# CMUAbstract/VINSat

Hardware: AMD Instinct MI355X
Metric: BA iterations/sec (500 poses, 50k landmarks) + final pose RMSE vs ref (higher is better)
Workload: dtype f64; 1 GPU; C3: 500-pose / 50000-observation window, 20-call schedule (10 landmark-only + 10 full); poses=500, observations=50000, windows_per_gpu=1, parallelism=replicas1, devices_visible=1, ranks_per_device=1

## Files before the change

### vinsat_amd/csrc/vba_api.hip

```cpp
#include "vba_context.h"

thread_local std::string g_err;

int fail(int code, const std::string& msg) {
    g_err = msg;
    return code;
}



void fill_params(StepParams& p, int iter, int initialize) {
    double alpha = 1.0 - (2.0 * ((double)iter / 5.0) - 1.0);
    alpha = std::min(std::max(alpha, 1.0), 2.0);
    const double it1 = (double)iter + 1.0;
    const double sigma = std::min(10000.0 * it1 * it1, 1000000.0);
    p.alpha = alpha;
    p.am2 = std::fabs(alpha - 2.0);
    p.expo = alpha / 2.0 - 1.0;
    p.alpha_is_2 = alpha == 2.0;
    p.sigma = sigma;
    p.sqrt_sigma = std::sqrt(sigma);
    p.initialize = initialize ? 1 : 0;
    p.iter = iter;
    p.pad = 0;
}

int check_window(vba_handle h, int window) {
    if (!h) return fail(VBA_EINVAL, "null handle");
    if (window < 0 || window >= h->W) return fail(VBA_EINVAL, "window index out of range");
    return VBA_OK;
}

int read_heads(vba_handle h) {
    HIPCHK(hipStreamSynchronize(h->stream));
    for (int w = 0; w < h->W; ++w)
        if (h->h_head[w].flags & 64u)
            return fail(VBA_ESTATE, "resident solve: a block of window " + std::to_string(w) + " timed out waiting for its producers (vba_set_fusion bits 5, 6)");
    return VBA_OK;
}

const volatile WinHead* head(vba_handle h, int w) { return h->h_head + w; }

hipError_t create_aux_stream(hipStream_t* s) {
    if (const char* m = std::getenv("VBA_AUX_CUMASK")) {
        const uint32_t word = (uint32_t)std::strtoul(m, nullptr, 16);
        uint32_t mask[8];
        for (auto& x : mask) x = word;
        return hipExtStreamCreateWithCUMask(s, 8, mask);
    }
    const char* e = std::getenv("VBA_AUX_PRIO");
    const int want = e ? std::atoi(e) : 0;
    if (want == 0) return hipStreamCreateWithFlags(s, hipStreamNonBlocking);
    int least = 0, greatest = 0;
    (void)hipDeviceGetStreamPriorityRange(&least, &greatest);
    return hipStreamCreateWithPriority(s, hipStreamNonBlocking, want > 0 ? greatest : least);
}

int settle(vba_handle h, bool boundary) {
    if (!h) return VBA_OK;
    if (!h->spec.valid) {
        if (boundary) h->prev_res_iter = -1;
        return VBA_OK;
    }
    HIPCHK(hipSetDevice(h->device));
    launch_reset_calls(h->V, h->stream);
    HIPCHK(hipGetLastError());
    HIPCHK(hipStreamSynchronize(h->stream));
    for (int w = 0; w < h->W; ++w) h->h_head[w].flags = 0;
    h->par = (h->chain_par0 + h->spec.c) & 1;
    h->carry_ok = 0;
    h->need_hist_reset = true;
    h->hist_dirty = false;
    h->spec.valid = false;
    h->spec_discards++;
    if (boundary && h->prev_res_iter >= 0) h->pred_iter[h->prev_res_iter & 63] = -2;
    h->prev_res_iter = -1;
    return VBA_OK;
}

int ready(vba_handle h) {
    for (int w = 0; w < h->W; ++w)
        if (!h->have_obs[w] || !h->have_win[w] || !h->have_state[w])
            return fail(VBA_ESTATE, "window " + std::to_string(w) + " is missing observations, pose constants or states");
    if (h->reg)
        for (int w = 0; w < h->W; ++w)
            if (!h->have_prior[w]) return fail(VBA_ESTATE, "window " + std::to_string(w) + " has no prior (vba_upload_prior)");
    return VBA_OK;
}



static int vba_set_accumulate_lanes(vba_handle h, int lanes);
static int vba_set_trial_tiles(vba_handle h, int tiles);
int vba_set_solver(vba_handle h, int chunk);

int vba_version(void) { return 230; }

const char* vba_last_error(void) { return g_err.c_str(); }

int vba_device_count(int* count) {
    if (!count) return fail(VBA_EINVAL, "null count");
    int c = 0;
    if (hipGetDeviceCount(&c) != hipSuccess) c = 0;
    *count = c;
    return VBA_OK;
}

constexpr int kLatWindowsCap = 192;
constexpr int kPartitionedWindowsMax = 1023;
static bool default_latency_mode(int windows, int64_t m_max) {
    const double x = m_max <= 50000 ? 0.7 : 0.46;
    return windows == 1 || (windows <= kLatWindowsCap && (double)windows <= 38.0 * std::pow(50000.0 / (double)m_max, x));
}
static int default_fusion(bool lat, int windows, int n_max, int64_t m_max) {
    const double rows = (double)windows * (double)m_max;
    if (windows == 1) return (lat && (m_max >= 150000 || n_max >= 1500)) ? 14 : 15;
    return !lat ? 15 : rows <= 175e3 ? 15 : rows <= 450e3 ? 14 : 12;
}

int vba_create(int device, int windows, int n_max, int64_t m_max, vba_handle* out) {
    return vba_create_mode(device, windows, n_max, m_max, -1, out);
}

int vba_create_mode(int device, int windows, int n_max, int64_t m_max, int mode, vba_handle* out) {
    if (!out) return fail(VBA_EINVAL, "null out");
    *out = nullptr;
    if (mode < -1 || mode > 1) return fail(VBA_EINVAL, "mode must be -1 (automatic), 0 (bandwidth-mode kernels) or 1 (latency-mode kernels)");
    const bool lat = mode == -1 ? default_latency_mode(windows, m_max) : mode == 1;
    if (windows < 1 || n_max < 2 || m_max < 1) return fail(VBA_EINVAL, "need windows >= 1, n_max >= 2, m_max >= 1");
    if (m_max > (int64_t)1 << 30) return fail(VBA_EINVAL, "m_max too large");
    int cnt = 0;
    if (hipGetDeviceCount(&cnt) != hipSuccess || cnt == 0) return fail(VBA_ENODEV, "no HIP device visible");
    if (device < 0 || device >= cnt) return fail(VBA_EINVAL, "device index out of range");
    HIPCHK(hipSetDevice(device));
    HIPCHK(configure_solver_device());
    vba_context* h = new (std::nothrow) vba_context();
    if (!h) return fail(VBA_ENOMEM, "host allocation failed");
    h->device = device;
    h->W = windows;
    h->n_max = n_max;
    h->m_max = m_max;
    const size_t W = windows, N = n_max, M = (size_t)m_max;
    const int nblk_obs = (int)((M + kObsBlock - 1) / kObsBlock);
    const int nblk_dyn = (int)((N + kObsBlock - 1) / kObsBlock);
    const int nblk_dyn16 = (int)((N - 1 + 14) / 15);
    const int trial_stride = nblk_obs + std::max(nblk_dyn, nblk_dyn16) + kLongCap;
    size_t bytes = 0;
    auto need = [&](size_t b) { bytes += ((b + 255) & ~size_t(255)) + 256; };
    need(W * 4); need(W * 4); need(W * sizeof(WinScalars));
    const size_t m_pad = (M + 31) & ~size_t(31);
    const size_t obs_stride = (6 * m_pad + m_pad / 2 + (N + 2) / 2 + 31) & ~size_t(31);
    need(W * obs_stride * 8);
    need(W * N * 10 * 8); need(W * N * 10 * 8);
    need(W * N * 4 * 8); need(W * N * 4 * 8); need(W * N * 4);
    const int nblk_pred = (int)((N * kDynLanes + 255) / 256);
    const int pred_stride = nblk_pred + kLongCap;
    need(W * 2 * pred_stride * 8); need(W * 2 * pred_stride * 8); need(W * 81 * 8);
    const size_t long_pool_cap = windows <= kLongPoolFewWindows ? kLongPoolFew : kLongPool;
    need(W * kLongCap * 4); need(W * 4); need(W * kLongCap * 4); need(W * 2 * long_pool_cap * 6 * 8);
    need(W * N * 36 * 8); need(W * N * 6 * 8);
    need(W * 2 * M * 8); need(2 * W * M * 8); need(W * 2 * M * 8); need(W * nblk_obs * 8); need(W * trial_stride * 8); need(W * nblk_obs * 8);
    need(W * kHistStride * 4);
    const int warm_shift = !lat ? 46 : (2 * m_max <= 300000 ? 44 : 43);
    int bucket_cap = 0;
    if (lat) {
        const double expect = 2.0 * (double)m_max * (warm_shift == 44 ? 0.0013 : 0.00065) * 6.0;
        bucket_cap = 256;
        while (bucket_cap < expect && bucket_cap < 4096) bucket_cap *= 2;
        need(W * 2 * (size_t)kSelBins * bucket_cap * 8);
    }
    const size_t per_pose = 2 * (21 + 6) + 2 * (6 + 36 + 6 + 1 + 3 + 9 + 9 + 9) + 243 + 9 + 81 + 9 + 9;
    need(W * N * per_pose * 8 + 16 * 256);
    need(W * N * 171 * 8);
    need(W * N * (171 + 171 + 81 + 9 + 9) * 8 + 6 * 256);
    need(W * N * (171 * 3 + 9) * 8 + 6 * 256);
    need(W * (N + 8) * 4);
    bytes += 1 << 16;
    if (hipMalloc(&h->arena.base, bytes) != hipSuccess) {
        delete h;
        return fail(VBA_ENOMEM, "hipMalloc of " + std::to_string(bytes) + " bytes failed");
    }
    h->arena.size = bytes;
    if (hipMemset(h->arena.base, 0, bytes) != hipSuccess || hipStreamSynchronize(nullptr) != hipSuccess) {
        hipFree(h->arena.base);
        delete h;
        return fail(VBA_EHIP, "hipMemset of the device arena failed");
    }
    Arena& A = h->arena;
    DevView& V = h->V;
    V.W = windows; V.n_max = n_max; V.m_max = m_max; V.nblk_obs = nblk_obs; V.nblk_dyn = nblk_dyn;
    V.n = h->d_n = A.take<int>(W);
    V.m = h->d_m = A.take<int>(W);
    V.sc = A.take<WinScalars>(W);
    h->d_obs = A.take<double>(W * obs_stride);
    h->m_pad = (int64_t)m_pad;
    V.obs_stride = (int64_t)obs_stride;
    V.ox = h->d_obs; V.oy = V.ox + m_pad; V.oz = V.oy + m_pad; V.ou = V.oz + m_pad; V.ov = V.ou + m_pad; V.oconf = V.ov + m_pad;
    V.opose = reinterpret_cast<const int*>(V.oconf + m_pad);
    V.pose_ptr = V.opose + m_pad;
    h->S[0] = A.take<double>(W * N * 10); h->S[1] = A.take<double>(W * N * 10);
    V.states = V.states_prev = h->S[0]; V.states_new = h->S[1];
    V.part_pred = A.take<double>(W * 2 * pred_stride); V.part_prior = A.take<double>(W * 2 * pred_stride); V.nblk_pred = nblk_pred;
    V.pred_stride = pred_stride;
    V.long_idx = h->d_long_idx = A.take<int>(W * kLongCap); V.n_long = h->d_n_long = A.take<int>(W);
    V.nblk_long = 0;
    V.long_off = h->d_long_off = A.take<int>(W * kLongCap);
    V.long_pool = A.take<double>(W * 2 * long_pool_cap * 6);
    V.long_pool_cap = (int)long_pool_cap;
    V.lastD = A.take<double>(W * 81);
    V.intr = h->d_intr = A.take<double>(W * N * 4);
    V.cumrot = h->d_cumrot = A.take<double>(W * N * 4);
    V.steps = h->d_steps = A.take<int>(W * N);
    V.prior_H = h->d_prior_H = A.take<double>(W * N * 36);
    V.prior_x = h->d_prior_x = A.take<double>(W * N * 6);
    V.reg = 0;
    V.absr = A.take<double>(W * 2 * M); V.wraw = h->wraw2 = A.take<double>(2 * W * M); V.ckeys = A.take<double>(W * 2 * M);
    V.acc_lanes = 8;
    V.part_init = A.take<double>(W * nblk_obs); V.part_trial = A.take<double>(W * trial_stride);
    V.trial_stride = trial_stride;
    V.part_next = A.take<double>(W * nblk_obs);
    V.hist = A.take<unsigned>(W * kHistStride);
    V.wbucket = bucket_cap ? A.take<double>(W * 2 * (size_t)kSelBins * bucket_cap) : nullptr;
    V.bucket_cap = bucket_cap;
    h->bucket_cap_alloc = bucket_cap;
    V.sel_inline = 0;
    V.Hraw = h->Hraw2 = A.take<double>(2 * W * N * 21); V.braw = h->braw2 = A.take<double>(2 * W * N * 6);
    V.xhat = h->dyn2[0] = A.take<double>(2 * W * N * 6); V.Phi = h->dyn2[1] = A.take<double>(2 * W * N * 36); V.rorb = h->dyn2[2] = A.take<double>(2 * W * N * 6);
    V.fatt = h->dyn2[3] = A.take<double>(2 * W * N); V.qgrad = h->dyn2[4] = A.take<double>(2 * W * N * 3);
    V.Hd = h->dyn2[5] = A.take<double>(2 * W * N * 9); V.Hu = h->dyn2[6] = A.take<double>(2 * W * N * 9); V.Hl = h->dyn2[7] = A.take<double>(2 * W * N * 9);
    V.bands = A.take<double>(W * N * 243); V.rhs = A.take<double>(W * N * 9);
    V.Xs = A.take<double>(W * N * 81); V.zs = A.take<double>(W * N * 9); V.dpose = A.take<double>(W * N * 9);
    V.p_max = n_max / 2 + 1;
    const size_t PM = V.p_max;
    V.csol = A.take<double>(W * N * 171);
    V.cL = A.take<double>(W * PM * 171); V.cR = A.take<double>(W * PM * 171);
    V.rXs = A.take<double>(W * PM * 81); V.rzs = A.take<double>(W * PM * 9); V.rx = A.take<double>(W * PM * 9);
    V.csol2 = A.take<double>(W * PM * 171); V.cL2 = A.take<double>(W * PM * 171); V.cR2 = A.take<double>(W * PM * 171);
    V.rx2 = A.take<double>(W * PM * 9);
    V.res_stride = n_max + 8;
    V.res_flags = A.take<unsigned>(W * (N + 8));
    V.resident = 0;
    V.m_total = 0; V.abs_all = nullptr; V.abs_all_count = 0;
    V.hop = 0; V.pivot = 0; V.call = -1; V.emit = 0; V.carry = 0; V.dyn_in_acc = 0;
    V.par = 0; V.fold = 0; V.redo = 0; V.fused_trial = 0; V.pending_only = 0; V.warm_force_miss = 0;
    V.lat = lat ? 1 : 0;
    V.trial_tiles = 1;
    V.warm_shift = warm_shift;
    V.chunk = 0; V.chunk2 = 0;
    {
        const void* must[] = {V.n, V.m, V.sc, V.ox, V.oy, V.oz, V.ou, V.ov, V.oconf, V.opose, V.pose_ptr, V.states,
                              V.states_new, V.states_prev, V.intr, V.cumrot, V.steps, V.prior_H, V.prior_x, V.absr, V.wraw, V.ckeys, V.part_init, V.part_next,
                              V.part_pred, V.part_prior, V.lastD, V.long_idx, V.n_long, V.long_off, V.long_pool,
                              V.part_trial, V.hist, V.Hraw, V.braw, V.xhat, V.Phi, V.rorb, V.fatt, V.qgrad, V.Hd, V.Hu, V.Hl,
                              V.bands, V.rhs, V.Xs, V.zs, V.dpose, V.csol, V.cL, V.cR, V.rXs, V.rzs, V.rx, V.csol2, V.cL2, V.cR2, V.rx2, V.res_flags};
        bool ok = A.used <= A.size;
        for (const void* q : must) ok = ok && q != nullptr;
        if (!ok) {
            hipFree(A.base);
            delete h;
            return fail(VBA_ENOMEM, "internal: device arena mis-carved");
        }
    }
    for (int k = 0; k < 64; ++k) h->pred_iter[k] = h->pred_init[k] = -1;
    h->V.host_states = nullptr;
    h->fusion = default_fusion(lat, windows, n_max, m_max);
    if ((windows == 1 && (hipEventCreateWithFlags(&h->ev_first, hipEventDisableTiming) != hipSuccess ||
                          hipHostMalloc((void**)&h->h_states_map, (size_t)2 * n_max * 10 * sizeof(double), hipHostMallocMapped | hipHostMallocCoherent) != hipSuccess ||
                          hipHostGetDevicePointer((void**)&h->V.host_states, h->h_states_map, 0) != hipSuccess)) ||
        hipStreamCreateWithFlags(&h->own_stream, hipStreamNonBlocking) != hipSuccess ||
        (!lat && create_aux_stream(&h->aux_stream) != hipSuccess) ||
        hipEventCreate(&h->ev0) != hipSuccess || hipEventCreate(&h->ev1) != hipSuccess ||
        hipEventCreateWithFlags(&h->ev_fork, hipEventDisableTiming) != hipSuccess ||
        hipEventCreateWithFlags(&h->ev_join, hipEventDisableTiming) != hipSuccess ||
        hipEventCreateWithFlags(&h->ev_stage, hipEventDisableTiming) != hipSuccess ||
        hipEventCreateWithFlags(&h->ev_up[0], hipEventDisableTiming) != hipSuccess ||
        hipEventCreateWithFlags(&h->ev_up[1], hipEventDisableTiming) != hipSuccess ||
        hipHostMalloc((void**)&h->h_up[0], std::max(obs_stride, 9 * N + 160) * sizeof(double), hipHostMallocDefault) != hipSuccess ||
        hipHostMalloc((void**)&h->h_up[1], std::max(obs_stride, 9 * N + 160) * sizeof(double), hipHostMallocDefault) != hipSuccess ||
        hipHostMalloc((void**)&h->h_stage, ((size_t)n_max * 10 + 1) * sizeof(double), hipHostMallocDefault) != hipSuccess ||
        hipHostMalloc((void**)&h->h_back, (size_t)n_max * 10 * sizeof(double) + sizeof(WinScalars), hipHostMallocDefault) != hipSuccess ||
        hipHostMalloc((void**)&h->h_head, W * sizeof(WinHead), hipHostMallocMapped | hipHostMallocCoherent) != hipSuccess ||
        hipHostGetDevicePointer((void**)&h->V.host_head, h->h_head, 0) != hipSuccess) {
        vba_destroy(h);
        return fail(VBA_EHIP, "stream/event/pinned allocation failed");
    }
    h->stream = h->own_stream;
    h->n.assign(W, 0); h->m.assign(W, 0); h->n_long.assign(W, 0);
    h->have_obs.assign(W, 0); h->have_win.assign(W, 0); h->have_state.assign(W, 0); h->have_prior.assign(W, 0);
    h->perm.resize(W);
    vba_set_accumulate_lanes(h, 0);
    vba_set_trial_tiles(h, 0);
    vba_set_solver(h, -1);
    h->warm_enabled = 1;
    h->fold_enabled = lat;
    if (const char* e = std::getenv("VBA_X_FOLD")) h->fold_enabled = std::atoi(e) != 0;
#ifdef VBA_VARIANTS
    if (const char* e = std::getenv("VBA_CR_LEVELS")) h->cr_levels = std::atoi(e) == 3 ? 3 : 2;
#endif
    *out = h;
    return VBA_OK;
}

int vba_has_variants(void) {
#ifdef VBA_VARIANTS
    return 1;
#else
    return 0;
#endif
}

int vba_get_mode(vba_handle h, int* mode, int* chunk) {
    if (!h) return fail(VBA_EINVAL, "null handle");
    if (mode) *mode = h->V.lat;
    if (chunk) *chunk = h->V.chunk;
    return VBA_OK;
}

int vba_destroy(vba_handle h) {
    if (!h) return VBA_OK;
    (void)settle(h);
    watch_stop(h);
    hipSetDevice(h->device);
    (void)vba_sh_comm_destroy(h);
    if (h->own_stream) { hipStreamSynchronize(h->own_stream); hipStreamDestroy(h->own_stream); }
    if (h->aux_stream) { hipStreamSynchronize(h->aux_stream); hipStreamDestroy(h->aux_stream); }
    for (hipEvent_t e : h->cprof.ev) if (e) hipEventDestroy(e);
    for (auto& ge : h->graphs) if (ge.exec) (void)hipGraphExecDestroy(ge.exec);
    if (h->ev_first) hipEventDestroy(h->ev_first);
    if (h->h_states_map) hipHostFree(h->h_states_map);
    if (h->ev_fork) hipEventDestroy(h->ev_fork);
    if (h->ev_join) hipEventDestroy(h->ev_join);
    if (h->ev0) hipEventDestroy(h->ev0);
    if (h->ev1) hipEventDestroy(h->ev1);
    if (h->ev_stage) hipEventDestroy(h->ev_stage);
    for (int k = 0; k < 2; ++k) {
        if (h->ev_up[k]) hipEventDestroy(h->ev_up[k]);
        if (h->h_up[k]) hipHostFree(h->h_up[k]);
    }
    if (h->h_stage) hipHostFree(h->h_stage);
    if (h->h_back) hipHostFree(h->h_back);
    if (h->h_head) hipHostFree(h->h_head);
    if (h->d_dbg) hipFree(h->d_dbg);
    for (QueryScratch* q : {&h->q_cov, &h->q_rel, &h->q_pow}) {
        if (q->d) hipFree(q->d);
        if (q->ev) hipEventDestroy(q->ev);
    }
    if (h->cov_ev0) hipEventDestroy(h->cov_ev0);
    if (h->arena.base) hipFree(h->arena.base);
    delete h;
    return VBA_OK;
}

int vba_set_solver2(vba_handle h, int chunk, int chunk2) {
    if (!h) return fail(VBA_EINVAL, "null handle");
    if (int rc_settle = settle(h)) return rc_settle;
    if (chunk < 2 || chunk > 60 || (chunk2 != 0 && chunk2 != -1 && (chunk2 < 2 || chunk2 > 60)))
        return fail(VBA_EINVAL, "chunk sizes must be in [2, 60] (chunk2 = 0: single level, -1: cyclic reduction)");
    if (chunk2 == -1 && (h->n_max + chunk - 1) / chunk - 1 > 128)
        return fail(VBA_EINVAL, "chunk2 = -1 needs at most 128 separators: chunk >= ceil(n_max / 129)");
    h->V.chunk = chunk;
    h->V.chunk2 = chunk2;
    h->no_pack = 0;
    return VBA_OK;
}

int vba_set_solver(vba_handle h, int chunk) {
    if (!h) return fail(VBA_EINVAL, "null handle");
    if (int rc_settle = settle(h)) return rc_settle;
    h->V.chunk2 = 0;
    if (chunk == -1) {
        h->no_pack = 0;
        if (h->W > kPartitionedWindowsMax || h->n_max < 8) { h->V.chunk = 0; return VBA_OK; }
        const int c64 = (h->n_max + 64) / 65, c128 = (h->n_max + 128) / 129;
        int c1 = std::max(std::min(c64, std::max(8, c128)), 2);
        if (!h->V.lat) c1 = std::max(c1, std::min(12, std::max(2, h->n_max / 3)));
        if (h->V.lat) c1 = std::max(c1, std::min(8, std::max(2, h->n_max / 3)));
        if (h->V.lat && h->W > 1) {
            int c = c1;
            while (c < 12 && (int64_t)h->W * ((h->n_max + c - 1) / c) > 1024) ++c;
            if ((int64_t)h->W * ((h->n_max + c - 1) / c) <= 1024) c1 = c;
        }
        if (c1 <= 60) {
            h->V.chunk = c1;
            h->V.chunk2 = -1;
        } else {
            const int c3 = std::min(std::max((int)std::ceil(std::cbrt((double)h->n_max)), 2), 60);
            h->V.chunk = c3;
            h->V.chunk2 = c3;
        }
        return VBA_OK;
    }
    if (chunk == -2) {
        h->V.chunk = 0;
        h->no_pack = 1;
        return VBA_OK;
    }
#ifndef VBA_VARIANTS
    if (chunk == -3) return fail(VBA_EINVAL, "three windows per wavefront (k_solve_packed) is a comparison variant that this build does not carry (make VARIANTS=1)");
#endif
    if (chunk == -3) {
        h->V.chunk = 0;
        h->no_pack = 0;
        h->pack_min = 3;
        return VBA_OK;
    }
    if (chunk < 0 || chunk == 1 || chunk > 60) return fail(VBA_EINVAL, "chunk must be -3, -2, -1, 0 or in [2, 60]");
    h->V.chunk = chunk;
    h->no_pack = 0;
    return VBA_OK;
}

int vba_set_integrator(vba_handle h, int hop100) {
    if (!h) return fail(VBA_EINVAL, "null handle");
    if (int rc_settle = settle(h)) return rc_settle;
    h->V.hop = hop100 ? 1 : 0;
    h->V.nblk_long = h->V.hop ? 0 : *std::max_element(h->n_long.begin(), h->n_long.end());
    return VBA_OK;
}

static int vba_set_accumulate_lanes(vba_handle h, int lanes) {
    if (!h) return fail(VBA_EINVAL, "null handle");
    if (int rc_settle = settle(h)) return rc_settle;
    if (lanes == 0) {
        const double avg = (double)h->m_max / (double)h->n_max;
        int G = 4;
        while (G < 64 && avg / G > 16.0) G *= 2;
        while (G < 64 && (int64_t)h->W * h->n_max * G * 2 <= 49152) G *= 2;
        lanes = G;
    }
    if (lanes != 4 && lanes != 8 && lanes != 16 && lanes != 32 && lanes != 64) return fail(VBA_EINVAL, "lanes must be 0, 4, 8, 16, 32 or 64");
    h->V.acc_lanes = lanes;
    return VBA_OK;
}

static int vba_set_trial_tiles(vba_handle h, int tiles) {
    if (!h) return fail(VBA_EINVAL, "null handle");
    if (int rc_settle = settle(h)) return rc_settle;
    if (tiles == 0) {
        const int64_t blocks = (int64_t)h->W * h->V.nblk_obs;
        tiles = blocks >= 600 ? 4 : (blocks >= 150 ? 2 : 1);
    }
    if (tiles != 1 && tiles != 2 && tiles != 4 && tiles != 8) return fail(VBA_EINVAL, "tiles must be 0 (automatic), 1, 2, 4 or 8");
    h->V.trial_tiles = tiles;
    return VBA_OK;
}

static int vba_set_key_carry(vba_handle h, int on) {
    if (!h) return fail(VBA_EINVAL, "null handle");
    if (int rc_settle = settle(h)) return rc_settle;
    h->carry_enabled = on != 0;
    h->carry_ok = false;
    return VBA_OK;
}

static int vba_set_fusion(vba_handle h, int mask) {
    if (!h) return fail(VBA_EINVAL, "null handle");
    if (int rc_settle = settle(h)) return rc_settle;
    if (mask < 0 || mask > 127) return fail(VBA_EINVAL, "mask must be in [0, 127]");
#ifndef VBA_VARIANTS
    if (mask & (16 | 32 | 64)) return fail(VBA_EINVAL, "mask bits 4 .. 6 select comparison variants that this build does not carry (make VARIANTS=1)");
#endif
    h->fusion = mask;
    h->fusion_auto = false;
    return VBA_OK;
}

static int vba_set_chunk_waves(vba_handle h, int waves) {
    if (!h) return fail(VBA_EINVAL, "null handle");
    if (int rc_settle = settle(h)) return rc_settle;
    if (waves != 1 && waves != 2) return fail(VBA_EINVAL, "waves must be 1 or 2");
    h->chunk_waves = waves;
    return VBA_OK;
}

static int vba_set_warm_select(vba_handle h, int on) {
    if (!h) return fail(VBA_EINVAL, "null handle");
    if (int rc_settle = settle(h)) return rc_settle;
    h->warm_enabled = on == 2 ? 2 : (on != 0);
    h->inline_select = on != 3;
    return VBA_OK;
}

static int vba_set_warm_shift(vba_handle h, int shift) {
    if (!h) return fail(VBA_EINVAL, "null handle");
    if (int rc_settle = settle(h)) return rc_settle;
    if (shift < 42 || shift > 51) return fail(VBA_EINVAL, "shift must be in [42, 51]");
    h->V.warm_shift = shift;
    h->carry_ok = 0;
    return VBA_OK;
}

static int vba_set_bucket_cap(vba_handle h, int cap) {
    if (!h) return fail(VBA_EINVAL, "null handle");
    if (int rc_settle = settle(h)) return rc_settle;
    if (!h->bucket_cap_alloc) return fail(VBA_ESTATE, "this handle has no bin buckets (16 windows or more)");
    if (cap != 0 && (cap < 8 || cap > h->bucket_cap_alloc)) return fail(VBA_EINVAL, "cap must be 0 (default) or in [8, allocated capacity]");
    h->V.bucket_cap = cap ? cap : h->bucket_cap_alloc;
    h->carry_ok = 0;
    return VBA_OK;
}

int vba_set_host_watch(vba_handle h, int slot, const void* live, const void* copy, int64_t bytes) {
    if (!h || slot < 0 || slot >= 8) return fail(VBA_EINVAL, "bad argument (8 watch slots)");
    if (live && (!copy || bytes < 1)) return fail(VBA_EINVAL, "a watched buffer needs its reference copy and a size");
    watch_quiesce(h);
    h->watch[slot].live = live;
    h->watch[slot].copy = live ? copy : nullptr;
    h->watch[slot].bytes = live ? (size_t)bytes : 0;
    return VBA_OK;
}

static int vba_set_pipeline(vba_handle h, int on) {
    if (!h) return fail(VBA_EINVAL, "null handle");
    if (int rc = settle(h)) return rc;
    h->pipeline = on != 0;
    return VBA_OK;
}

int vba_pipeline_stats(vba_handle h, int* hits, int* discards) {
    if (!h) return fail(VBA_EINVAL, "null handle");
    if (hits) *hits = h->spec_hits;
    if (discards) *discards = h->spec_discards;
    return VBA_OK;
}

int vba_warm_select_misses(vba_handle h, int* count) {
    if (!h || !count) return fail(VBA_EINVAL, "null argument");
    *count = h->warm_misses;
    return VBA_OK;
}

static int vba_set_jacobian_f32(vba_handle h, int on) {
    if (!h) return fail(VBA_EINVAL, "null handle");
    if (int rc_settle = settle(h)) return rc_settle;
    if (on != 0 && on != 1) return fail(VBA_EINVAL, "jacobian_f32 must be 0 (fp64, default) or 1 (fp32)");
    h->V.jac_f32 = on;
    return VBA_OK;
}

static int vba_set_pivoting(vba_handle h, int always) {
    if (!h) return fail(VBA_EINVAL, "null handle");
    if (int rc_settle = settle(h)) return rc_settle;
    h->pivot_mode = always ? 1 : 0;
    return VBA_OK;
}

int vba_solver_fallbacks(vba_handle h, int* count) {
    if (!h || !count) return fail(VBA_EINVAL, "null argument");
    *count = h->fallbacks;
    return VBA_OK;
}

int vba_set_stream(vba_handle h, void* hip_stream, int external) {
    if (!h) return fail(VBA_EINVAL, "null handle");
    if (int rc_settle = settle(h)) return rc_settle;
    hipStreamSynchronize(h->stream);
    h->stream = external ? (hipStream_t)hip_stream : h->own_stream;
    return VBA_OK;
}

int vba_upload_observations(vba_handle h, int window, int n, int64_t m, const double* xyz, const double* uv,
                            const double* conf, const int64_t* ii) {
    if (int rc = check_window(h, window)) return rc;
    if (int rc_settle = settle(h, true)) return rc_settle;
    if (!xyz || !uv || !conf || !ii) return fail(VBA_EINVAL, "null observation array");
    h->carry_ok = false;
    if (n < 2 || n > h->n_max) return fail(VBA_EINVAL, "n out of range (need 2 <= n <= n_max)");
    if (m < 1 || m > h->m_max) return fail(VBA_EINVAL, "m out of range (need 1 <= m <= m_max)");
    if (h->have_win[window] && h->n[window] != n) { h->have_win[window] = 0; h->have_state[window] = 0; h->have_prior[window] = 0; }
    HIPCHK(hipSetDevice(h->device));
    std::vector<int> ptr(n + 1, 0);
    for (int64_t k = 0; k < m; ++k) {
        if (ii[k] < 0 || ii[k] >= n) return fail(VBA_EINVAL, "ii[" + std::to_string(k) + "] outside [0, n)");
        ptr[ii[k] + 1]++;
    }
    for (int i = 0; i < n; ++i) ptr[i + 1] += ptr[i];
    std::vector<int64_t>& perm = h->perm[window];
    perm.assign(m, 0);
    if (!h->perm_stale.empty()) h->perm_stale[window] = 1;
    {
        std::vector<int> cur(ptr.begin(), ptr.end() - 1);
        for (int64_t k = 0; k < m; ++k) perm[cur[ii[k]]++] = k;
    }
    const int ub = h->up_next;
    h->up_next ^= 1;
    HIPCHK(hipEventSynchronize(h->ev_up[ub]));
    double* blk = h->h_up[ub];
    const size_t mp = (size_t)h->m_pad;
    double *x = blk, *y = x + mp, *z = y + mp, *u = z + mp, *v = u + mp, *c = v + mp;
    int* pose = reinterpret_cast<int*>(c + mp);
    int* cptr = pose + mp;
    for (int64_t s = 0; s < m; ++s) {
        const int64_t k = perm[s];
        x[s] = xyz[3 * k]; y[s] = xyz[3 * k + 1]; z[s] = xyz[3 * k + 2];
        u[s] = uv[2 * k]; v[s] = uv[2 * k + 1];
        c[s] = conf[k];
        pose[s] = (int)ii[k];
    }
    std::memcpy(cptr, ptr.data(), (size_t)(n + 1) * sizeof(int));
    const int mi = (int)m;
    const size_t used = (size_t)(reinterpret_cast<char*>(cptr + n + 1) - reinterpret_cast<char*>(blk));
    HIPCHK(hipMemcpyAsync(h->d_obs + (size_t)window * h->V.obs_stride, blk, used, hipMemcpyHostToDevice, h->stream));
    HIPCHK(hipEventRecord(h->ev_up[ub], h->stream));
    launch_set_counts(h->V, window, n, mi, h->stream);
    HIPCHK(hipGetLastError());
    h->n[window] = n;
    h->m[window] = mi;
    h->have_obs[window] = 1;
    h->V.n_min = *std::min_element(h->n.begin(), h->n.end());
    return VBA_OK;
}

int vba_upload_window(vba_handle h, int window, int n, const double* intrinsics, const double* cumrot_last,
                      const int64_t* time_idx) {
    if (int rc = check_window(h, window)) return rc;
    if (int rc_settle = settle(h, true)) return rc_settle;
    if (!intrinsics || !cumrot_last || !time_idx) return fail(VBA_EINVAL, "null pose-constant array");
    h->carry_ok = false;
    if (n < 2 || n > h->n_max) return fail(VBA_EINVAL, "n out of range (need 2 <= n <= n_max)");
    if (h->have_obs[window] && h->n[window] != n) { h->have_obs[window] = 0; h->have_state[window] = 0; h->have_prior[window] = 0; }
    HIPCHK(hipSetDevice(h->device));
    std::vector<int> steps(n);
    for (int i = 0; i + 1 < n; ++i) {
        const int64_t d = time_idx[i + 1] - time_idx[i];
        if (d < 1) return fail(VBA_EINVAL, "time_idx must be strictly increasing");
        if (d > VBA_MAX_GAP) return fail(VBA_EINVAL, "time_idx: a gap longer than VBA_MAX_GAP (2^20 s)");
        steps[i] = (int)d;
    }
    steps[n - 1] = 1;
    int long_list[2 * kLongCap + 1];
    int nl = 0, pool_used = 0;
    for (int i = 0; i + 1 < n && nl < kLongCap; ++i)
        if (steps[i] > kLongGap) {
            const int need_states = long_pool_states(long_plan(steps[i]));
            if (pool_used + need_states > h->V.long_pool_cap) continue;
            long_list[kLongCap + 1 + nl] = pool_used;
            pool_used += need_states;
            long_list[nl++] = i;
            steps[i] = -steps[i];
        }
    long_list[kLongCap] = nl;
    const size_t pb = (size_t)window * h->n_max;
    const int ub = h->up_next;
    h->up_next ^= 1;
    HIPCHK(hipEventSynchronize(h->ev_up[ub]));
    double* blk = h->h_up[ub];
    std::memcpy(blk, intrinsics, (size_t)n * 32);
    std::memcpy(blk + (size_t)n * 4, cumrot_last, (size_t)n * 32);
    std::memcpy(blk + (size_t)n * 8, steps.data(), (size_t)n * 4);
    double* lblk = blk + (size_t)n * 8 + (size_t)(n + 1) / 2;
    std::memcpy(lblk, long_list, sizeof(long_list));
    HIPCHK(hipMemcpyAsync(h->d_intr + pb * 4, blk, (size_t)n * 32, hipMemcpyHostToDevice, h->stream));
    HIPCHK(hipMemcpyAsync(h->d_cumrot + pb * 4, blk + (size_t)n * 4, (size_t)n * 32, hipMemcpyHostToDevice, h->stream));
    HIPCHK(hipMemcpyAsync(h->d_steps + pb, blk + (size_t)n * 8, (size_t)n * 4, hipMemcpyHostToDevice, h->stream));
    if (nl) {
        HIPCHK(hipMemcpyAsync(h->d_long_idx + (size_t)window * kLongCap, lblk, (size_t)nl * 4, hipMemcpyHostToDevice, h->stream));
        HIPCHK(hipMemcpyAsync(h->d_long_off + (size_t)window * kLongCap, reinterpret_cast<const int*>(lblk) + kLongCap + 1, (size_t)nl * 4,
                              hipMemcpyHostToDevice, h->stream));
    }
    HIPCHK(hipMemcpyAsync(h->d_n_long + window, reinterpret_cast<const int*>(lblk) + kLongCap, 4, hipMemcpyHostToDevice, h->stream));
    if (nl || h->n_long[window])
        HIPCHK(hipMemsetAsync(h->V.long_pool + (size_t)window * 2 * h->V.long_pool_cap * 6, 0xFF,
                              (size_t)2 * h->V.long_pool_cap * 6 * sizeof(double), h->stream));
    HIPCHK(hipEventRecord(h->ev_up[ub], h->stream));
    h->n_long[window] = nl;
    h->V.nblk_long = h->V.hop ? 0 : *std::max_element(h->n_long.begin(), h->n_long.end());
    launch_set_counts(h->V, window, n, -1, h->stream);
    HIPCHK(hipGetLastError());
    h->n[window] = n;
    h->have_win[window] = 1;
    return VBA_OK;
}

int vba_upload_prior(vba_handle h, int window, int n, const double* states_prior, const double* hessian_state) {
    if (int rc = check_window(h, window)) return rc;
    if (int rc_settle = settle(h, true)) return rc_settle;
    if (!states_prior || !hessian_state) return fail(VBA_EINVAL, "null prior array");
    if (!h->have_obs[window] && !h->have_win[window]) return fail(VBA_ESTATE, "upload the window before its prior");
    if (n != h->n[window]) return fail(VBA_EINVAL, "the prior needs one row per pose of the window");
    HIPCHK(hipSetDevice(h->device));
    std::vector<double> xp((size_t)n * 6);
    for (int i = 0; i < n; ++i) {
        const double* s = states_prior + (size_t)i * 10;
        double* o = xp.data() + (size_t)i * 6;
        o[0] = s[0]; o[1] = s[1]; o[2] = s[2]; o[3] = s[7]; o[4] = s[8]; o[5] = s[9];
    }
    HIPCHK(hipStreamSynchronize(h->stream));
    const size_t pb = (size_t)window * h->n_max;
    HIPCHK(hipMemcpy(h->d_prior_x + pb * 6, xp.data(), xp.size() * 8, hipMemcpyHostToDevice));
    HIPCHK(hipMemcpy(h->d_prior_H + pb * 36, hessian_state, (size_t)n * 36 * 8, hipMemcpyHostToDevice));
    h->have_prior[window] = 1;
    return VBA_OK;
}

int vba_set_prior(vba_handle h, int on) {
    if (!h) return fail(VBA_EINVAL, "null handle");
    h->reg = on != 0;
    return VBA_OK;
}

int vba_set_states(vba_handle h, int window, const double* states, double lamda) {
    if (!h) return fail(VBA_EINVAL, "null handle");
    if (int rc_settle = settle(h, true)) return rc_settle;
    if (!states) return fail(VBA_EINVAL, "null states");
    h->carry_ok = 0;
    double* S = h->S[h->par];
    if (window == -1) {
        const int n = h->n[0];
        for (int w = 0; w < h->W; ++w) {
            if (!h->have_obs[w] && !h->have_win[w]) return fail(VBA_ESTATE, "upload the windows before their states");
            if (h->n[w] != n) return fail(VBA_EINVAL, "window = -1 needs equal pose counts");
        }
        HIPCHK(hipSetDevice(h->device));
        HIPCHK(hipEventSynchronize(h->ev_stage));
        std::memcpy(h->h_stage, states, (size_t)n * 80);
        HIPCHK(hipMemcpyAsync(S, h->h_stage, (size_t)n * 80, hipMemcpyHostToDevice, h->stream));
        HIPCHK(hipEventRecord(h->ev_stage, h->stream));
        DevView V = h->V;
        V.states = S;
        V.par = h->par;
        launch_broadcast_states(V, n, lamda, h->stream);
        HIPCHK(hipGetLastError());
        for (int w = 0; w < h->W; ++w) h->have_state[w] = 1;
        return VBA_OK;
    }
    if (int rc = check_window(h, window)) return rc;
    if (!h->have_obs[window] && !h->have_win[window]) return fail(VBA_ESTATE, "upload the window before its states");
    HIPCHK(hipSetDevice(h->device));
    const int n = h->n[window];
    HIPCHK(hipEventSynchronize(h->ev_stage));
    std::memcpy(h->h_stage, states, (size_t)n * 80);
    h->h_stage[(size_t)h->n_max * 10] = lamda;
    HIPCHK(hipMemcpyAsync(S + (size_t)window * h->n_max * 10, h->h_stage, (size_t)n * 80, hipMemcpyHostToDevice, h->stream));
    HIPCHK(hipMemcpyAsync(&h->V.sc[window].lam[h->par], h->h_stage + (size_t)h->n_max * 10, 8, hipMemcpyHostToDevice, h->stream));
    HIPCHK(hipEventRecord(h->ev_stage, h->stream));
    h->have_state[window] = 1;
    return VBA_OK;
}

void unpack_scalars(const WinScalars* sc, int par, double* lamda, double* last_hessian, int* n_trials, unsigned* flags) {
    if (lamda) *lamda = sc->lam[par];
    if (last_hessian) std::memcpy(last_hessian, sc->last_hessian, 81 * 8);
    if (n_trials) *n_trials = sc->n_trials;
    if (flags) *flags = sc->fl[par ^ 1] & 7u;
}

int vba_get_states(vba_handle h, int window, double* states, double* lamda, double* last_hessian, int* n_trials,
                   unsigned* flags) {
    if (int rc = check_window(h, window)) return rc;
    if (int rc_settle = settle(h)) return rc_settle;
    if (!h->have_state[window]) return fail(VBA_ESTATE, "no states uploaded");
    HIPCHK(hipSetDevice(h->device));
    const int n = h->n[window];
    WinScalars* sc = reinterpret_cast<WinScalars*>(h->h_back + (size_t)h->n_max * 10);
    if (states) HIPCHK(hipMemcpyAsync(h->h_back, h->S[h->par] + (size_t)window * h->n_max * 10, (size_t)n * 80, hipMemcpyDeviceToHost, h->stream));
    HIPCHK(hipMemcpyAsync(sc, h->V.sc + window, sizeof(WinScalars), hipMemcpyDeviceToHost, h->stream));
    HIPCHK(hipStreamSynchronize(h->stream));
    if (states) std::memcpy(states, h->h_back, (size_t)n * 80);
    unpack_scalars(sc, h->par, lamda, last_hessian, n_trials, flags);
    return VBA_OK;
}

int vba_set_states_all(vba_handle h, const double* states, const double* lamda) {
    if (!h) return fail(VBA_EINVAL, "null handle");
    if (int rc_settle = settle(h, true)) return rc_settle;
    if (!states || !lamda) return fail(VBA_EINVAL, "null states / lamda");
    for (int w = 0; w < h->W; ++w)
        if (!h->have_obs[w] && !h->have_win[w]) return fail(VBA_ESTATE, "upload the windows before their states");
    HIPCHK(hipSetDevice(h->device));
    h->carry_ok = 0;
    const size_t per = (size_t)h->n_max * 10;
    HIPCHK(hipStreamSynchronize(h->stream));
    HIPCHK(hipMemcpy(h->S[h->par], states, (size_t)h->W * per * sizeof(double), hipMemcpyHostToDevice));
    std::vector<WinScalars> sc((size_t)h->W);
    HIPCHK(hipMemcpy(sc.data(), h->V.sc, sc.size() * sizeof(WinScalars), hipMemcpyDeviceToHost));
    for (int w = 0; w < h->W; ++w) sc[w].lam[h->par] = lamda[w];
    HIPCHK(hipMemcpy(h->V.sc, sc.data(), sc.size() * sizeof(WinScalars), hipMemcpyHostToDevice));
    for (int w = 0; w < h->W; ++w) h->have_state[w] = 1;
    return VBA_OK;
}

int vba_get_states_all(vba_handle h, double* states, double* lamda, double* last_hessian, int* n_trials, unsigned* flags) {
    if (!h) return fail(VBA_EINVAL, "null handle");
    if (int rc_settle = settle(h)) return rc_settle;
    for (int w = 0; w < h->W; ++w)
        if (!h->have_state[w]) return fail(VBA_ESTATE, "no states uploaded");
    HIPCHK(hipSetDevice(h->device));
    HIPCHK(hipStreamSynchronize(h->stream));
    const size_t per = (size_t)h->n_max * 10;
    if (states) HIPCHK(hipMemcpy(states, h->S[h->par], (size_t)h->W * per * sizeof(double), hipMemcpyDeviceToHost));
    std::vector<WinScalars> sc((size_t)h->W);
    HIPCHK(hipMemcpy(sc.data(), h->V.sc, sc.size() * sizeof(WinScalars), hipMemcpyDeviceToHost));
    for (int w = 0; w < h->W; ++w)
        unpack_scalars(&sc[w], h->par, lamda ? lamda + w : nullptr, last_hessian ? last_hessian + (size_t)w * 81 : nullptr,
                       n_trials ? n_trials + w : nullptr, flags ? flags + w : nullptr);
    return VBA_OK;
}


int vba_set_option(vba_handle h, int option, int value) {
    switch (option) {
        case VBA_OPT_ACCUMULATE_LANES: return vba_set_accumulate_lanes(h, value);
        case VBA_OPT_TRIAL_TILES: return vba_set_trial_tiles(h, value);
        case VBA_OPT_KEY_CARRY: return vba_set_key_carry(h, value);
        case VBA_OPT_WARM_SELECT: return vba_set_warm_select(h, value);
        case VBA_OPT_WARM_SHIFT: return vba_set_warm_shift(h, value);
        case VBA_OPT_BUCKET_CAP: return vba_set_bucket_cap(h, value);
        case VBA_OPT_FUSION: return vba_set_fusion(h, value);
        case VBA_OPT_CHUNK_WAVES: return vba_set_chunk_waves(h, value);
        case VBA_OPT_PIVOTING: return vba_set_pivoting(h, value);
        case VBA_OPT_PIPELINE: return vba_set_pipeline(h, value);
        case VBA_OPT_SCHEDULE_GRAPH: return vba_set_schedule_graph(h, value);
        case VBA_OPT_CHAIN_PROFILE: return vba_set_chain_profile(h, value);
        case VBA_OPT_JACOBIAN_F32: return vba_set_jacobian_f32(h, value);
        default: return fail(VBA_EINVAL, "unknown option (VBA_OPT_*)");
    }
}

int vba_last_step_ms(vba_handle h, float* ms) {
    if (!h || !ms) return fail(VBA_EINVAL, "null argument");
    if (!h->stepped) return fail(VBA_ESTATE, "no step has run");
    *ms = h->last_ms;
    return VBA_OK;
}

int vba_debug_fetch(vba_handle h, int window, int what, double* out, int64_t capacity, int64_t* count) {
    if (int rc = check_window(h, window)) return rc;
    if (int rc_settle = settle(h)) return rc_settle;
    if (!out || !count) return fail(VBA_EINVAL, "null output");
    if (!h->stepped) return fail(VBA_ESTATE, "no step has run");
    if (h->last_pipelined)
        return fail(VBA_ESTATE, "the last call was a pipelined vba_iterate_resident: the call speculated behind it has reused its scratch "
                                "(maximum weight, step, trial states); switch the pipeline off (vba_set_pipeline(h, 0)) to inspect intermediates");
    HIPCHK(hipSetDevice(h->device));
    HIPCHK(hipStreamSynchronize(h->stream));
    const int n = h->n[window];
    const int64_t m = h->m[window];
    const size_t pb = (size_t)window * h->n_max;
    DevView V;
    {
        CallSpec c;
        c.iter = h->last_iter; c.initialize = h->last_init; c.call = -1; c.par = h->par ^ 1;
        view_for_call(h, V, c);
    }
    auto copy = [&](const double* src, int64_t cnt) -> int {
        if (cnt > capacity) return fail(VBA_EINVAL, "debug buffer too small");
        HIPCHK(hipMemcpy(out, src, cnt * 8, hipMemcpyDeviceToHost));
        *count = cnt;
        return VBA_OK;
    };
    WinScalars sc;
    HIPCHK(hipMemcpy(&sc, V.sc + window, sizeof(sc), hipMemcpyDeviceToHost));
    double wmax;
    std::memcpy(&wmax, &sc.wmax_bits[V.par], 8);
    switch (what) {
#ifdef VBA_RESIDENT_STAMPS
        case 100:
            return copy(V.cR2 + (size_t)window * V.res_stride * 4, (int64_t)V.res_stride * 4);
        case 102: {
            if (capacity < 64) return fail(VBA_EINVAL, "debug buffer too small");
            fetch_ostamps(reinterpret_cast<unsigned long long*>(out));
            *count = 64;
            return VBA_OK;
        }
        case 101: {
            if (capacity < 128) return fail(VBA_EINVAL, "debug buffer too small");
            fetch_kstamps(reinterpret_cast<unsigned long long*>(out));
            *count = 128;
            return VBA_OK;
        }
#endif
        case VBA_DBG_EST:
        case VBA_DBG_WEIGHT:
        case VBA_DBG_JG: {
            const int64_t per = what == VBA_DBG_EST ? 2 : (what == VBA_DBG_JG ? 12 : 1);
            if (m * per > capacity) return fail(VBA_EINVAL, "debug buffer too small");
            const size_t need = (size_t)m * 15 * 8;
            if (h->dbg_cap < need) {
                if (h->d_dbg) hipFree(h->d_dbg);
                h->d_dbg = nullptr;
                h->dbg_cap = 0;
                HIPCHK(hipMalloc(&h->d_dbg, need));
                h->dbg_cap = need;
            }
            double* est = h->d_dbg;
            double* J = est + 2 * m;
            double* wt = J + 12 * m;
            launch_debug_project(V, window, (int)m, est, J, wt, h->stream);
            HIPCHK(hipGetLastError());
            HIPCHK(hipStreamSynchronize(h->stream));
            std::vector<double> tmp((size_t)m * per);
            const double* src = what == VBA_DBG_EST ? est : (what == VBA_DBG_JG ? J : wt);
            HIPCHK(hipMemcpy(tmp.data(), src, (size_t)m * per * 8, hipMemcpyDeviceToHost));
            const std::vector<int64_t>& perm = h->perm[window];
            for (int64_t s = 0; s < m; ++s) std::memcpy(out + perm[s] * per, tmp.data() + s * per, per * 8);
            *count = m * per;
            return VBA_OK;
        }
        case VBA_DBG_H: {
            if ((int64_t)n * 36 > capacity) return fail(VBA_EINVAL, "debug buffer too small");
            std::vector<double> tmp((size_t)n * 21);
            HIPCHK(hipMemcpy(tmp.data(), V.Hraw + pb * 21, (size_t)n * 21 * 8, hipMemcpyDeviceToHost));
            for (int i = 0; i < n; ++i)
                for (int a = 0; a < 6; ++a)
                    for (int b = 0; b < 6; ++b) out[(size_t)i * 36 + a * 6 + b] = tmp[(size_t)i * 21 + sym6(a, b)] / wmax;
            *count = (int64_t)n * 36;
            return VBA_OK;
        }
        case VBA_DBG_B: {
            if (int rc = copy(V.braw + pb * 6, (int64_t)n * 6)) return rc;
            for (int64_t k = 0; k < (int64_t)n * 6; ++k) out[k] /= wmax;
            return VBA_OK;
        }
        case VBA_DBG_PHI: return copy(V.Phi + pb * 36, (int64_t)n * 36);
        case VBA_DBG_RPRED: {
            if ((int64_t)(n - 1) * 7 > capacity) return fail(VBA_EINVAL, "debug buffer too small");
            std::vector<double> ro((size_t)n * 6), fa(n);
            HIPCHK(hipMemcpy(ro.data(), V.rorb + pb * 6, (size_t)n * 48, hipMemcpyDeviceToHost));
            HIPCHK(hipMemcpy(fa.data(), V.fatt + pb, (size_t)n * 8, hipMemcpyDeviceToHost));
            for (int i = 0; i < n - 1; ++i) {
                for (int r = 0; r < 6; ++r) out[(size_t)i * 7 + r] = ro[(size_t)i * 6 + r];
                out[(size_t)i * 7 + 6] = fa[i];
            }
            *count = (int64_t)(n - 1) * 7;
            return VBA_OK;
        }
        case VBA_DBG_QGRAD: return copy(V.qgrad + pb * 3, (int64_t)n * 3);
        case VBA_DBG_HQ: {
            if ((int64_t)n * 27 > capacity) return fail(VBA_EINVAL, "debug buffer too small");
            std::vector<double> d((size_t)n * 9), u((size_t)n * 9), l((size_t)n * 9);
            HIPCHK(hipMemcpy(d.data(), V.Hd + pb * 9, (size_t)n * 72, hipMemcpyDeviceToHost));
            HIPCHK(hipMemcpy(u.data(), V.Hu + pb * 9, (size_t)n * 72, hipMemcpyDeviceToHost));
            HIPCHK(hipMemcpy(l.data(), V.Hl + pb * 9, (size_t)n * 72, hipMemcpyDeviceToHost));
            for (int i = 0; i < n; ++i)
                for (int k = 0; k < 9; ++k) {
                    out[(size_t)i * 27 + k] = l[(size_t)i * 9 + k];
                    out[(size_t)i * 27 + 9 + k] = d[(size_t)i * 9 + k];
                    out[(size_t)i * 27 + 18 + k] = u[(size_t)i * 9 + k];
                }
            *count = (int64_t)n * 27;
            return VBA_OK;
        }
        case VBA_DBG_BANDS: {
            if (!std::getenv("VBA_DBG_RAW_BANDS")) launch_assemble(V, 0, h->stream);
            HIPCHK(hipGetLastError());
            HIPCHK(hipStreamSynchronize(h->stream));
            if (int rc = copy(V.bands + pb * 243, (int64_t)n * 243)) return rc;
            if (h->last_init) {
                for (int i = 0; i < n; ++i) {
                    std::memset(out + (size_t)i * 243, 0, 81 * 8);
                    std::memset(out + (size_t)i * 243 + 162, 0, 81 * 8);
                }
            }
            return VBA_OK;
        }
        case VBA_DBG_RHS: {
            if (!std::getenv("VBA_DBG_RAW_BANDS")) launch_assemble(V, 0, h->stream);
            HIPCHK(hipGetLastError());
            HIPCHK(hipStreamSynchronize(h->stream));
            return copy(V.rhs + pb * 9, (int64_t)n * 9);
        }
        case VBA_DBG_DPOSE: return copy(V.dpose + pb * 9, (int64_t)n * 9);
        case VBA_DBG_SCALARS: {
            if (capacity < 8) return fail(VBA_EINVAL, "debug buffer too small");
            StepParams p;
            fill_params(p, h->last_iter, h->last_init);
            out[0] = sc.c_obs; out[1] = wmax; out[2] = sc.init_residual; out[3] = sc.trial_residual;
            out[4] = sc.lam32; out[5] = p.sigma; out[6] = p.alpha; out[7] = (double)sc.n_trials;
            *count = 8;
            return VBA_OK;
        }
        default: return fail(VBA_EINVAL, "unknown debug selector");
    }
}
```

### vinsat_amd/csrc/vba_context.h

```cpp
#pragma once
#include <algorithm>
#include <atomic>
#include <chrono>
#include <cmath>
#include <condition_variable>
#include <mutex>
#include <thread>
#include <cstdio>
#include <cstdlib>
#include <cstring>
#include <new>
#include <string>
#include <vector>

#include <dlfcn.h>
#include <unistd.h>
#include <rccl/rccl.h>

#include "../../include/vinsat_ba.h"
#include "vba_device.h"
#include "vba_launch.h"
#include "vba_query_layout.h"

using namespace vba;

#pragma GCC visibility push(hidden)
extern thread_local std::string g_err;
int fail(int code, const std::string& msg);
#define HIPCHK(expr)                                                                                   \
    do {                                                                                               \
        hipError_t e_ = (expr);                                                                        \
        if (e_ != hipSuccess)                                                                          \
            return fail(VBA_EHIP, std::string(#expr) + ": " + hipGetErrorString(e_));                  \
    } while (0)

struct Arena {
    char* base = nullptr;
    size_t size = 0, used = 0;
    template <class T>
    T* take(size_t count) {
        used = (used + 255) & ~size_t(255);
        T* p = reinterpret_cast<T*>(base + used);
        used += count * sizeof(T);
        return p;
    }
};

struct QueryScratch {
    void* d = nullptr;
    size_t cap = 0;
    hipEvent_t ev = nullptr;
    float ms = 0.f;
    bool ran = false;
};

struct vba_context {
    int device = 0;
    int W = 0, n_max = 0;
    int64_t m_max = 0;
    hipStream_t own_stream = nullptr, stream = nullptr, aux_stream = nullptr;
    hipEvent_t ev0 = nullptr, ev1 = nullptr, ev_fork = nullptr, ev_join = nullptr;
    Arena arena;
    DevView V{};
    int *d_n = nullptr, *d_m = nullptr, *d_steps = nullptr;
    int *d_long_idx = nullptr, *d_n_long = nullptr, *d_long_off = nullptr;
    std::vector<int> n_long;
    double *wraw2 = nullptr, *Hraw2 = nullptr, *braw2 = nullptr;
    double* dyn2[8] = {};
    double* d_obs = nullptr;
    int64_t m_pad = 0;
    double *d_intr = nullptr, *d_cumrot = nullptr;
    double* h_up[2] = {nullptr, nullptr};
    hipEvent_t ev_up[2] = {nullptr, nullptr};
    int up_next = 0;
    WinHead* h_head = nullptr;
    double* h_stage = nullptr;
    double* h_back = nullptr;
    bool back_valid = false;
    double* S[2] = {nullptr, nullptr};
    int par = 0;
    bool need_hist_reset = false;
    hipEvent_t ev_stage = nullptr;
    std::vector<int> n, m;
    std::vector<char> have_obs, have_win, have_state, have_prior;
    bool reg = false;
    double *d_prior_H = nullptr, *d_prior_x = nullptr;
    std::vector<std::vector<int64_t>> perm;
    float last_ms = 0.f;
    bool stepped = false;
    int carry_ok = 0;
    bool carry_enabled = true;
    bool hist_dirty = false;
    bool fold_enabled = true;
    int warm_enabled = 1;
    int last_iter = 0, last_init = 0;
    int sh_pivot = 0;
    bool sh_rode = false, sh_bands_ready = false;
    struct ShComm {
        void* dl = nullptr;
        ncclComm_t comm = nullptr;
        int nranks = 0, rank = 0;
        ncclResult_t (*all_gather)(const void*, void*, size_t, ncclDataType_t, ncclComm_t, hipStream_t) = nullptr;
        ncclResult_t (*comm_destroy)(ncclComm_t) = nullptr;
        const char* (*error_string)(ncclResult_t) = nullptr;
        double* buf = nullptr;
        int64_t m_total = 0, m_pad = 0;
        int n = 0;
        int m_local = -1;
        int protocol = 1;
        ncclResult_t (*group_start)() = nullptr;
        ncclResult_t (*group_end)() = nullptr;
        double* buf2 = nullptr;
        int lenA = 0, lenB = 0, n2 = 0, nbo2 = 0, nbd2 = 0, cap2 = 0;
        double *sendA[2] = {nullptr, nullptr}, *recvA = nullptr, *sendB = nullptr, *recvB = nullptr;
        bool carried = false;
        int carried_par = 0;
        long fallbacks_miss = 0, fallbacks_lm = 0;
        double *abs_local = nullptr, *abs_all = nullptr, *partial_local = nullptr, *partial_all = nullptr, *trial_local = nullptr, *trial_all = nullptr;
    } shc;
    int pack_min = 1 << 30;
    int no_pack = 0;
    int pivot_mode = 0;
    int fallbacks = 0;
    int inline_select = 1;
    int chunk_waves = 2;
    int cr_levels = 2;
    int fusion = 15;
    bool fusion_auto = true;
    struct GraphEntry { std::vector<unsigned long long> key; std::vector<unsigned char> views; hipGraphExec_t exec = nullptr; };
    std::vector<GraphEntry> graphs;
    bool graph_broken = false;
    bool graph_enabled = true;
    long graph_replays = 0, graph_captures = 0;
    int bucket_cap_alloc = 0;
    int warm_misses = 0;
    double* d_dbg = nullptr;
    size_t dbg_cap = 0;
    QueryScratch q_cov;
    QueryScratch q_rel;
    QueryScratch q_pow;
    hipEvent_t cov_ev0 = nullptr;
    bool sharded = false;
    std::vector<char> perm_stale;
    struct Spec { bool valid = false; int iter = 0, init = 0; bool reg = false; int c = 0; } spec;
    int chain_par0 = 0;
    int pred_iter[64], pred_init[64];
    int prev_res_iter = -1;
    int pipeline = 1;
    bool last_pipelined = false;
    int spec_hits = 0, spec_discards = 0;
    struct Watch { const void* live = nullptr; const void* copy = nullptr; size_t bytes = 0; } watch[8];
    struct WatchWorker {
        std::thread th;
        std::mutex m;
        std::condition_variable cv;
        unsigned long long seq = 0;
        bool quit = false;
        std::atomic<unsigned long long> done_seq{0};
        bool changed = false;
        bool started = false;
        pid_t owner = 0;
    } ww;
    struct ChainProf {
        bool on = false;
        std::vector<hipEvent_t> ev;
        double ms[3] = {0.0, 0.0, 0.0};
        int64_t launches[3] = {0, 0, 0};
    } cprof;
    double* h_states_map = nullptr;
    hipEvent_t ev_first = nullptr;
};

void fill_params(StepParams& p, int iter, int initialize);
int check_window(vba_handle h, int window);
int read_heads(vba_handle h);
const volatile WinHead* head(vba_handle h, int w);
hipError_t create_aux_stream(hipStream_t* s);
int settle(vba_handle h, bool boundary = false);
int ready(vba_handle h);
void unpack_scalars(const WinScalars* sc, int par, double* lamda, double* last_hessian, int* n_trials, unsigned* flags);

struct CallSpec {
    bool host_out = false;
    int iter = 0, initialize = 0;
    int call = -1;
    int par = 0;
    int carry = 0;
    int emit = 0;
    bool fold = false;
    bool prof = false;
};

struct CallCtx {
    DevView V;
    hipEvent_t after_first = nullptr;
    bool fuse_assemble = false;
    bool assembled = false;
    bool bands_ready = false;
};

void view_for_call(vba_handle h, DevView& V, const CallSpec& c);
int enqueue_front(vba_handle h, CallCtx& C, const CallSpec& c, bool exact_repeat, hipEvent_t* ev);
void enqueue_trial(vba_handle h, CallCtx& C, const CallSpec& c, bool first, hipEvent_t ev_solve = nullptr, int solve_redo = -1);
int step_impl(vba_handle h, int iter, int initialize, float* prof, bool emit = true, int readback = -1);
void watch_stop(vba_handle h);
void watch_quiesce(vba_handle h);
int vba_set_schedule_graph(vba_handle h, int on);
int vba_set_chain_profile(vba_handle h, int on);

struct CovQuery {
    DevView V;
    double* diag = nullptr;
    double* sup = nullptr;
    unsigned* flags = nullptr;
};
int cov_begin(vba_handle h, int iter, const char* who);
int cov_build_invert(vba_handle h, int iter, int damped, CovQuery& q);
int query_reserve(vba_handle h, QueryScratch& q, size_t bytes, const char* what);
int query_finish(vba_handle h, QueryScratch& q);
int query_last_ms(vba_handle h, QueryScratch vba_context::*q, float* ms, const char* none_ran);

int rel_device_perm(vba_handle h, const int** d_perm);
int query_copy_out(double* out, const double* dev, size_t W, size_t stride, const std::vector<int>& used, size_t per);
#pragma GCC visibility pop
```

### vinsat_amd/csrc/vba_launch.h

```cpp
#pragma once
#include <hip/hip_runtime.h>

#include "vba_device.h"

namespace vba {

void launch_obs_residual(const DevView& V, double* abs_out, hipStream_t s);
void launch_select(const DevView& V, bool with_digit0, hipStream_t s);
void launch_select_warm(const DevView& V, hipStream_t s);
void launch_select_finish(const DevView& V, hipStream_t s);
void launch_obs_accumulate(const DevView& V, hipStream_t s);
void launch_trial(const DevView& V, hipStream_t s);
void launch_clear_hist(const DevView& V, int which, hipStream_t s);
void launch_reset_calls(const DevView& V, hipStream_t s);
void launch_set_counts(const DevView& V, int w, int n, int m, hipStream_t s);
void launch_broadcast_states(const DevView& V, int n, double lamda, hipStream_t s);
void launch_debug_project(const DevView& V, int w, int m, double* est, double* J, double* wt, hipStream_t s);

void launch_sh_clear_miss(const DevView& V, hipStream_t s);
void launch_sh_front(const DevView& V, const double* gathered, int ranks, int slot_len, double* bucket_out, int do_fold, int do_resolve, hipStream_t s);

void launch_dynamics(const DevView& V, hipStream_t s);
void launch_assemble(const DevView& V, int fuse_init_solve, hipStream_t s);

void launch_long_factor(const DevView& V, hipStream_t s);
void launch_long_trial(const DevView& V, hipStream_t s);

void launch_solve(const DevView& V, int initialize, hipStream_t s);
#ifdef VBA_RESIDENT_STAMPS
void fetch_kstamps(unsigned long long* out);
void fetch_ostamps(unsigned long long* out);
#endif
hipError_t configure_solver_device();
bool solve_forms_blocks(const DevView& V);
void launch_decide(const DevView& V, const double* trial_all, int ranks, hipStream_t s);

void launch_shard_pack(const DevView& V, double* partial_out, hipStream_t s);
void launch_shard_reduce(const DevView& V, const double* partial_all, int ranks, hipStream_t s, int with_sum = 1);
void launch_shard_trial_sum(const DevView& V, double* trial_local, hipStream_t s);

}
```

### vinsat_amd/csrc/vba_obs.hip

```cpp
#include "vba_decide.h"
#include <cstdlib>
#include "vba_device.h"
#include "vba_dyn_body.h"
#include "vba_launch.h"
#include "vba_step.h"

namespace vba {

__device__ __forceinline__ void begin_call_scalars(WinScalars& sc, int par, bool keep_wmax = false) {
    sc.done = 0;
    sc.n_trials = 0;
    sc.fl[par] = 0u;
    if (!keep_wmax) sc.wmax_bits[par] = 0ull;
    sc.sum_abs_rpred = 0.0;
}

template <bool HIST0>
__global__ __launch_bounds__(kObsBlock) void k_obs_residual(DevView V, double* abs_out ) {
    __shared__ double red[kObsBlock / 64];
    __shared__ unsigned lh[HIST0 ? 1024 : 1];
    const int w = blockIdx.y;
    VBA_SKIP_CALL(V, w);
    const int m = V.m[w];
    const size_t ob = (size_t)w * V.obs_stride;
    const size_t mb = (size_t)w * V.m_max;
    const int k = blockIdx.x * kObsBlock + threadIdx.x;
    if (HIST0) {
        for (int b = threadIdx.x; b < 1024; b += kObsBlock) lh[b] = 0u;
        __syncthreads();
    }
    double s = 0.0;
    if (k < m) {
        const int pose = V.opose[2 * ob + k];
        const size_t pb = (size_t)w * V.n_max + pose;
        PoseCam pc;
        pose_camera(V.states + pb * 10, V.intr + pb * 4, pc);
        double u, v, cam[3], d;
        project(pc, V.ox[ob + k], V.oy[ob + k], V.oz[ob + k], u, v, cam, d);
        const double ru = fabs(V.ou[ob + k] - u), rv = fabs(V.ov[ob + k] - v);
        double* ab = abs_out ? abs_out : V.absr + 2 * mb;
        reinterpret_cast<double2*>(ab)[k] = make_double2(ru, rv);
        s = ru + rv;
        if (HIST0) {
            atomicAdd(&lh[(unsigned)(f64_bits(ru) >> 53) & 1023u], 1u);
            atomicAdd(&lh[(unsigned)(f64_bits(rv) >> 53) & 1023u], 1u);
        }
    }
    const double t = block_sum<kObsBlock>(s, red);
    if (threadIdx.x == 0) V.part_init[(size_t)w * V.nblk_obs + blockIdx.x] = t;
    if (blockIdx.x == 0 && threadIdx.x == 0) {
        begin_call_scalars(V.sc[w], V.par);
        V.sc[w].sel_cnt = 0u;
    }
    if (HIST0) {
        unsigned* hist = hist0_of(V, w, V.par);
        for (int b = threadIdx.x; b < 1024; b += kObsBlock) {
            const unsigned c = lh[b];
            if (c) atomicAdd(&hist[b], c);
        }
        if (blockIdx.x == 0 && threadIdx.x == 0) {
            V.sc[w].sel_prefix[0] = 0ull;
            V.sc[w].sel_rank[0] = (2 * (long long)m - 1) / 2;
        }
    }
}

template <int P, bool COMPACT, int ITEMS>
__global__ __launch_bounds__(256) void k_select_pass(DevView V) {
    __shared__ unsigned lh[kSelBins];
    __shared__ unsigned lds_u[260];
    __shared__ double red[kObsBlock / 64];
    const int w = blockIdx.y;
    VBA_SKIP_CALL(V, w);
    const double* keys = V.abs_all ? V.abs_all : V.absr + 2 * (size_t)w * V.m_max;
    const int64_t count = V.abs_all ? V.abs_all_count : 2 * (int64_t)V.m[w];
    if (P == 1 && V.carry && blockIdx.x == 0 && threadIdx.x == 0) {
        begin_call_scalars(V.sc[w], V.par);
        V.sc[w].sel_cnt = 0u;
    }
    if (P == 1 && !V.carry && V.m_total == 0 && blockIdx.x == 0) {
        const double* pi = V.part_init + (size_t)w * V.nblk_obs;
        double s_init = 0.0;
        for (int b = threadIdx.x; b < V.nblk_obs; b += 256) s_init += pi[b];
        const double tot = block_sum<256>(s_init, red);
        if (threadIdx.x == 0) V.sc[w].sum_in[V.par] = tot;
    }
    if ((int64_t)blockIdx.x * 256 * ITEMS >= count) return;
    auto digit_hist = [&](int d) { return d == 0 ? hist0_of(V, w, V.par) : histd_of(V, w, d); };
    constexpr int nbins = 1 << sel_width(P);
    for (int b = threadIdx.x; b < nbins; b += 256) lh[b] = 0u;
    constexpr bool PRELOAD = ITEMS <= 8;
    constexpr int PAIRS = ITEMS / 2;
    const double2* keys2 = reinterpret_cast<const double2*>(keys);
    const int64_t npair = count / 2;
    double2 pk[PRELOAD ? PAIRS : 1];
    if (PRELOAD) {
#pragma unroll
        for (int it = 0; it < PAIRS; ++it) {
            const int64_t idx = ((int64_t)blockIdx.x * PAIRS + it) * 256 + threadIdx.x;
            pk[it] = idx < npair ? keys2[idx] : make_double2(0.0, 0.0);
        }
    }
    unsigned long long prefix = 0ull;
    long long rank = ((V.m_total ? 2 * V.m_total : count) - 1) / 2;
    if (P > 0) {
        constexpr int Q = P > 0 ? P - 1 : 0;
        select_resolve(digit_hist(Q), 1 << sel_width(Q), sel_width(Q), V.sc[w].sel_prefix[Q], V.sc[w].sel_rank[Q],
                       prefix, rank, lds_u);
    } else {
        __syncthreads();
    }
    if (blockIdx.x == 0 && threadIdx.x == 0) {
        V.sc[w].sel_prefix[P] = prefix;
        V.sc[w].sel_rank[P] = rank;
        if (COMPACT) V.sc[w].sel_mode = 0;
    }
    auto take = [&](unsigned long long key, bool have) {
        bool match = have;
        if (P > 0) match = have && (key >> sel_shift(P > 0 ? P - 1 : 0)) == prefix;
        if (match) atomicAdd(&lh[(unsigned)(key >> sel_shift(P)) & (nbins - 1)], 1u);
        if (COMPACT) {
            const unsigned long long mask = __ballot(match);
            if (mask) {
                const int lane = threadIdx.x & 63;
                const int leader = __ffsll((long long)mask) - 1;
                unsigned base = 0;
                if (lane == leader) base = atomicAdd(&V.sc[w].sel_cnt, (unsigned)__popcll(mask));
                base = (unsigned)__builtin_amdgcn_readlane((int)base, leader);
                if (match) {
                    const unsigned off = (unsigned)__popcll(mask & ((1ull << lane) - 1ull));
                    if ((int64_t)base + off < 2 * V.m_max) V.ckeys[2 * (size_t)w * V.m_max + base + off] = bits_f64(key);
                }
            }
        }
    };
#pragma unroll 8
    for (int it = 0; it < PAIRS; ++it) {
        const int64_t idx = ((int64_t)blockIdx.x * PAIRS + it) * 256 + threadIdx.x;
        const bool have = idx < npair;
        const double2 kk = PRELOAD ? pk[it] : (have ? keys2[idx] : make_double2(0.0, 0.0));
        take(f64_bits(kk.x), have);
        take(f64_bits(kk.y), have);
    }
    __syncthreads();
    unsigned* hist_out = digit_hist(P);
    for (int b = threadIdx.x; b < nbins; b += 256) {
        const unsigned c = lh[b];
        if (c) atomicAdd(&hist_out[b], c);
    }
}

enum { kWarmSkip = 0, kWarmHit = 1, kWarmMiss = 2 };

__device__ __forceinline__ bool fold_decide(const DevView& V, int w, double (*red)[4], DecideOut& d) {
    d = decide_eval(V, w, V.par ^ 1, V.prev, 0, 0.0, nullptr, 0, red);
    return d.accept && !(d.flags & (2u | 8u | 32u));
}
__device__ __forceinline__ DecideIn fold_load(const DevView& V, int w) { return decide_load(V, w, V.par ^ 1, V.prev, 0); }
__device__ __forceinline__ bool fold_decide_loaded(const DevView& V, int w, const DecideIn& in, double (*red)[4], DecideOut& d) {
    d = decide_finish(V, w, in, V.prev, 0, 0.0, nullptr, 0, red);
    return d.accept && !(d.flags & (2u | 8u | 32u));
}
__device__ __forceinline__ void fold_commit(const DevView& V, int w, const DecideOut& d) {
    WinScalars& sc = V.sc[w];
    const int t = threadIdx.x, par = V.par;
    const double lam32 = sc.lam32;
    if (t < 81) {
        const double hv = V.lastD[(size_t)w * 81 + t] + ((t / 9 == t % 9) ? lam32 : 0.0);
        sc.last_hessian[t] = hv;
        if (V.host_states) V.host_head[w].last_hessian[t] = hv;
    }
    if (t == 0) {
        sc.lam[par] = d.lam_out;
        sc.sum_in[par] = d.sum_next;
        sc.init_residual = d.init_residual;
        sc.trial_residual = d.residual;
        sc.call_idx = V.call;
        WinHead& hh = V.host_head[w];
        hh.lamda = d.lam_out;
        hh.trial_residual = d.residual;
        hh.n_trials = 1;
        hh.flags = d.flags;
        hh.done = 1;
        hh.call_idx = V.call;
    }
}
__device__ __forceinline__ void front_commit(const DevView& V, int w, bool hit, unsigned bin, long long rank, unsigned in_bin, bool inline_select) {
    WinScalars& sc = V.sc[w];
    const int par = V.par;
    begin_call_scalars(sc, par, inline_select);
    if (hit) {
        sc.sel_mode = 1;
        sc.sel_rank[2] = rank;
        sc.warm_base = sc.warm_lo[par] + ((unsigned long long)(bin - 1u) << V.warm_shift);
        if (inline_select) sc.sel_cnt = in_bin;
    } else {
        sc.miss = 1;
        sc.fl[par] = 32u;
        V.host_head[w].flags = 32u;
        V.host_head[w].done = 0;
    }
}
__device__ __forceinline__ bool front_resolve(const DevView& V, int w, const unsigned (&hloc)[8], long long list_cap, unsigned* lds_u,
                                              unsigned& bin, long long& rank, unsigned& in_bin) {
    const int64_t count = 2 * (int64_t)V.m[w];
    const unsigned long long lo = V.sc[w].warm_lo[V.par];
    unsigned long long prefix;
    select_resolve_loaded(hloc, kSelBins, 11, 0ull, (count - 1) / 2, prefix, rank, lds_u, &in_bin);
    bin = (unsigned)prefix;
    return lo != ~0ull && bin >= 1u && bin <= 2046u && (int64_t)in_bin <= list_cap && !V.warm_force_miss;
}

__device__ __forceinline__ int warm_front(const DevView& V, int w, bool fold_here, bool inline_select, long long list_cap,
                                          double (*red)[4], unsigned* lds_u, unsigned& bin_out, long long& rank_out,
                                          unsigned& in_bin_out) {
    unsigned hloc[8];
    select_load(hist0_of(V, w, V.par), kSelBins, hloc);
    if (fold_here) {
        DecideOut d;
        if (!fold_decide(V, w, red, d)) return kWarmSkip;
        if (blockIdx.x == 0) fold_commit(V, w, d);
    }
    const bool hit = front_resolve(V, w, hloc, list_cap, lds_u, bin_out, rank_out, in_bin_out);
    if (blockIdx.x == 0 && threadIdx.x == 0) front_commit(V, w, hit, bin_out, rank_out, in_bin_out, inline_select);
    return hit ? kWarmHit : kWarmMiss;
}

template <int ITEMS>
__global__ __launch_bounds__(256) void k_select_warm(DevView V) {
    __shared__ unsigned lds_u[260];
    __shared__ double red[5][4];
    const int w = blockIdx.y;
    WinScalars& sc = V.sc[w];
    const int t = threadIdx.x;
    const bool fold_here = V.call >= 0 && V.fold && sc.pending == V.call - 1 && sc.call_idx == V.call - 1;
    if (!fold_here) VBA_SKIP_CALL(V, w);
    const double* keys = V.absr + 2 * (size_t)w * V.m_max;
    const int64_t count = 2 * (int64_t)V.m[w];
    if ((int64_t)blockIdx.x * 256 * ITEMS >= count) return;
    constexpr bool PRELOAD = ITEMS <= 8;
    constexpr int PAIRS = ITEMS / 2;
    const double2* keys2 = reinterpret_cast<const double2*>(keys);
    const int64_t npair = count / 2;
    double2 pk[PAIRS];
#pragma unroll
    for (int it = 0; it < PAIRS; ++it) {
        const int64_t idx = ((int64_t)blockIdx.x * PAIRS + it) * 256 + t;
        pk[it] = idx < npair ? keys2[idx] : make_double2(0.0, 0.0);
    }
    const unsigned long long lo = sc.warm_lo[V.par];
    unsigned bin, in_bin;
    long long rank;
    if (warm_front(V, w, fold_here, false, 2 * V.m_max, red, lds_u, bin, rank, in_bin) != kWarmHit) return;
    if constexpr (!PRELOAD) {
        double2 (&kk)[PAIRS] = pk;
        unsigned long long mbits = 0ull;
#pragma unroll
        for (int it = 0; it < PAIRS; ++it) {
            const int64_t idx = ((int64_t)blockIdx.x * PAIRS + it) * 256 + t;
            const bool have = idx < npair;
            if (have && warm_bin(f64_bits(kk[it].x), lo, V.warm_shift) == bin) mbits |= 1ull << (2 * it);
            if (have && warm_bin(f64_bits(kk[it].y), lo, V.warm_shift) == bin) mbits |= 2ull << (2 * it);
        }
        const unsigned mine = (unsigned)__popcll(mbits);
        const unsigned inc = wave_inclusive_scan_u32(mine);
        __syncthreads();
        if ((t & 63) == 63) lds_u[t >> 6] = inc;
        __syncthreads();
        if (t == 0) {
            const unsigned total = lds_u[0] + lds_u[1] + lds_u[2] + lds_u[3];
            lds_u[4] = total ? atomicAdd(&sc.sel_cnt, total) : 0u;
        }
        __syncthreads();
        unsigned at = lds_u[4] + inc - mine;
        for (int q = 0; q < (t >> 6); ++q) at += lds_u[q];
        double* list = V.ckeys + 2 * (size_t)w * V.m_max;
#pragma unroll
        for (int it = 0; it < PAIRS; ++it) {
            if (mbits & (1ull << (2 * it))) list[at++] = kk[it].x;
            if (mbits & (2ull << (2 * it))) list[at++] = kk[it].y;
        }
        return;
    }
    auto take = [&](unsigned long long key, bool have) {
        const bool match = have && warm_bin(key, lo, V.warm_shift) == bin;
        const unsigned long long mask = __ballot(match);
        if (mask) {
            const int lane = t & 63;
            const int leader = __ffsll((long long)mask) - 1;
            unsigned base = 0;
            if (lane == leader) base = atomicAdd(&sc.sel_cnt, (unsigned)__popcll(mask));
            base = (unsigned)__builtin_amdgcn_readlane((int)base, leader);
            if (match) V.ckeys[2 * (size_t)w * V.m_max + base + (unsigned)__popcll(mask & ((1ull << lane) - 1ull))] = bits_f64(key);
        }
    };
    if constexpr (PRELOAD) {
#pragma unroll 8
        for (int it = 0; it < PAIRS; ++it) {
            const int64_t idx = ((int64_t)blockIdx.x * PAIRS + it) * 256 + t;
            const bool have = idx < npair;
            take(f64_bits(pk[it].x), have);
            take(f64_bits(pk[it].y), have);
        }
// ... 655 lines not shown
                    kbin[2 * tl] = warm_bin(f64_bits(ru), wlo, V.warm_shift);
                    kbin[2 * tl + 1] = warm_bin(f64_bits(rv), wlo, V.warm_shift);
                    if (V.wbucket) {
                        kslot[2 * tl] = atomicAdd(&lh[kbin[2 * tl]], 1u);
                        kslot[2 * tl + 1] = atomicAdd(&lh[kbin[2 * tl + 1]], 1u);
                        kkey[2 * tl] = ru;
                        kkey[2 * tl + 1] = rv;
                        kvalid[tl] = true;
                    } else {
                        atomicAdd(&lh[kbin[2 * tl]], 1u);
                        atomicAdd(&lh[kbin[2 * tl + 1]], 1u);
                    }
                } else {
                    atomicAdd(&lh[(unsigned)(f64_bits(ru) >> 53) & 1023u], 1u);
                    atomicAdd(&lh[(unsigned)(f64_bits(rv) >> 53) & 1023u], 1u);
                }
            }
        }
    }
    } else if (PART != 1) {
        const int db = part_slot - V.nblk_obs;
        const bool reg = V.reg && !prm.initialize;
        int i;
        bool edge_thread;
        bool pose_thread;
        const double* st;
        const double* sn;
        if (FUSED == 0) {
            i = db * kObsBlock + tid;
            edge_thread = pose_thread = true;
            st = V.states_new + (sb + i) * 10;
            sn = st + 10;
        } else {
            const int i0 = db * kEdgesPerBlock16;
            const int j = i0 + grp;
            i = j;
            edge_thread = l16 == 0 && grp < kEdgesPerBlock16;
            pose_thread = l16 == 0 && (grp < kEdgesPerBlock16 || j / kEdgesPerBlock16 >= V.nblk_dyn);
            if (FORM && fz) {
                const bool live = j < n;
                double o[10], d9[9];
                unsigned b2 = 0u;
                pose_trial_state_group<FORM ? FUSED : 1>(V, w, j, live, l16, gbase, inv_wmax, lam32, o, d9, b2);
                bad = b2;
                if (live && l16 == 0) {
#pragma unroll
                    for (int r = 0; r < 10; ++r) snew[(size_t)grp * 10 + r] = o[r];
                    if (pose_thread) {
#pragma unroll
                        for (int r = 0; r < 10; ++r) V.states_new[(sb + j) * 10 + r] = o[r];
#pragma unroll
                        for (int r = 0; r < 9; ++r) V.dpose[(sb + j) * 9 + r] = d9[r];
                        if (V.host_states) {
#pragma unroll
                            for (int r = 0; r < 10; ++r) V.host_states[((size_t)par * V.n_max + j) * 10 + r] = o[r];
                        }
                    }
                }
                if (FUSED == 1 && live && j == n - 1) {
                    const double* H = V.Hraw + (sb + j) * 21;
                    for (int e = l16; e < 81; e += 16) {
                        const int a = e / 9, c = e % 9;
                        V.lastD[(size_t)w * 81 + e] = (a < 6 && c < 6) ? H[sym6(a, c)] * inv_wmax : 0.0;
                    }
                }
                __syncthreads();
                st = snew + (size_t)grp * 10;
                sn = st + 10;
            } else {
                st = V.states_new + (sb + j) * 10;
                sn = st + 10;
            }
        }
        if (edge_thread && !prm.initialize && i < n - 1) {
            double x[6] = {st[0], st[1], st[2], st[7], st[8], st[9]};
            const int steps = V.steps[sb + i];
            if (steps > 0 || V.hop) {
                propagate_gap<false>(x, nullptr, abs(steps), V.hop);
                s = fabs(x[0] - sn[0]) + fabs(x[1] - sn[1]) + fabs(x[2] - sn[2]) +
                    fabs((x[3] - sn[7]) * kVelCoeff) + fabs((x[4] - sn[8]) * kVelCoeff) + fabs((x[5] - sn[9]) * kVelCoeff);
            }
            double att = fabs(attitude_residual(st + 3, V.cumrot + (sb + i) * 4, sn + 3));
            if (reg) att *= 1.0 / kQuatCoeff;
            s += att;
            s *= prm.sqrt_sigma;
        }
        if (reg && pose_thread && i < n) {
            double r6[6];
            prior_residual(V.prior_H + (sb + i) * 36, V.prior_x + (sb + i) * 6, st, r6);
            s += fabs(r6[0]) + fabs(r6[1]) + fabs(r6[2]) + fabs(r6[3]) + fabs(r6[4]) + fabs(r6[5]);
        }
    }
    VBA_OSTAMP(4);
    constexpr int kBinsPerThread = kSelBins / kObsBlock;
    static_assert(kSelBins % kObsBlock == 0, "bins per thread");
    unsigned bb[kBinsPerThread] = {};
    const bool bucketing = EMIT == 2 && PART == 0 && obs_block && V.wbucket;
    if (bucketing) {
        __syncthreads();
        unsigned* hist = hist0_of(V, w, par ^ 1);
#pragma unroll
        for (int q = 0; q < kBinsPerThread; ++q) {
            const unsigned c = lh[tid + q * kObsBlock];
            bb[q] = c ? atomicAdd(&hist[tid + q * kObsBlock], c) : 0u;
        }
    }
    VBA_OSTAMP(5);
    if (TILES > 1 && obs_block) {
#pragma unroll
        for (int tl = 0; tl < TILES; ++tl) {
            const double a = wave_sum(s_tile[tl]), r2 = wave_sum(sraw_tile[tl]);
            if ((tid & 63) == 0) {
                redt[(2 * tl) * (kObsBlock / 64) + (tid >> 6)] = a;
                redt[(2 * tl + 1) * (kObsBlock / 64) + (tid >> 6)] = r2;
            }
        }
        __syncthreads();
        if (tid < 2 * TILES && part_slot + tid / 2 < V.nblk_obs) {
            double t = 0.0;
#pragma unroll
            for (int i = 0; i < kObsBlock / 64; ++i) t += redt[tid * (kObsBlock / 64) + i];
            if (tid & 1) { if (EMIT) V.part_next[(size_t)w * V.nblk_obs + part_slot + tid / 2] = t; }
            else V.part_trial[(size_t)w * V.trial_stride + part_slot + tid / 2] = t;
        }
    } else {
        const double t = block_sum<kObsBlock>(s, red);
        if (tid == 0) V.part_trial[(size_t)w * V.trial_stride + part_slot] = t;
    }
    VBA_OSTAMP(6);
    if (FORM && !obs_block) {
        const unsigned long long bp = __ballot(bad & 1u), bn = __ballot(bad & 2u);
        if ((tid & 63) == 0 && (bp || bn)) atomicOr(&sc.fl[par], (bp ? (8u | 16u) : 0u) | (bn ? 2u : 0u));
    }
    if (EMIT && PART != 2 && obs_block) {
        if (TILES == 1) {
            const double t_raw = block_sum<kObsBlock>(s_raw, red);
            if (tid == 0) V.part_next[(size_t)w * V.nblk_obs + part_slot] = t_raw;
        }
        unsigned* hist = hist0_of(V, w, par ^ 1);
        if (bucketing) {
#pragma unroll
            for (int q = 0; q < kBinsPerThread; ++q) lh[tid + q * kObsBlock] = bb[q];
            __syncthreads();
            VBA_OSTAMP(7);
            double* pool = V.wbucket + ((size_t)w * 2 + (par ^ 1)) * kSelBins * (size_t)V.bucket_cap;
#pragma unroll
            for (int q = 0; q < 2 * TILES; ++q) {
                if (kvalid[q / 2]) {
                    const unsigned slot = lh[kbin[q]] + kslot[q];
                    if (kbin[q] >= 1u && kbin[q] <= 2046u && slot < (unsigned)V.bucket_cap) pool[(size_t)kbin[q] * V.bucket_cap + slot] = kkey[q];
                }
            }
            VBA_OSTAMP(8);
        } else {
            for (int b = tid; b < kEmitBins; b += kObsBlock) {
                const unsigned c = lh[b];
                if (c) atomicAdd(&hist[b], c);
            }
        }
    }
}

__global__ __launch_bounds__(256) void k_sh_front(DevView V, const double* gathered, int ranks, int slot_len, double* bucket_out, int do_fold,
                                                  int do_resolve) {
    __shared__ unsigned lds_u[260];
    __shared__ double red[5][4];
    __shared__ unsigned over;
    const int w = 0, t = threadIdx.x;
    WinScalars& sc = V.sc[w];
    const int off_next = 1024, off_trial = 1024 + V.nblk_obs;
    const int seen_call = sc.call_idx, seen_pending = sc.pending, seen_miss = sc.miss;
    const int pc = V.par ^ 1;
    const double lam_in = sc.lam[pc], so_in = sc.sum_in[pc];
    const unsigned fl_in = sc.fl[pc];
    const unsigned long long lo = sc.warm_lo[V.par];
    double s_next = 0.0, s_trial = 0.0, s_pred = 0.0;
    for (int q = 0; q < ranks; ++q) {
        const double* slot = gathered + (size_t)q * slot_len;
        for (int b = t; b < V.nblk_obs; b += 256) { s_next += slot[off_next + b]; s_trial += slot[off_trial + b]; }
    }
    for (int b = t; b < V.nblk_dyn + (V.prev.initialize ? 0 : V.nblk_long); b += 256) s_trial += gathered[off_trial + V.nblk_obs + b];
    if (do_fold && !V.prev.initialize) {
        const double* pp = V.part_pred + ((size_t)w * 2 + pc) * V.pred_stride;
        for (int b = t; b < V.nblk_pred + V.nblk_long; b += 256) s_pred += pp[b];
    }
    unsigned hl[8], mine[8];
    if (do_resolve) {
        const uint4* own4 = reinterpret_cast<const uint4*>(hist0_of(V, w, V.par)) + 2 * t;
        const uint4 o0 = own4[0], o1 = own4[1];
        mine[0] = o0.x; mine[1] = o0.y; mine[2] = o0.z; mine[3] = o0.w; mine[4] = o1.x; mine[5] = o1.y; mine[6] = o1.z; mine[7] = o1.w;
#pragma unroll
        for (int j = 0; j < 8; ++j) hl[j] = 0u;
        for (int q = 0; q < ranks; ++q) {
            const uint4* g4 = reinterpret_cast<const uint4*>(gathered + (size_t)q * slot_len) + 2 * t;
            const uint4 g0 = g4[0], g1 = g4[1];
            hl[0] += g0.x; hl[1] += g0.y; hl[2] += g0.z; hl[3] += g0.w; hl[4] += g1.x; hl[5] += g1.y; hl[6] += g1.z; hl[7] += g1.w;
        }
    }
    if (do_fold) {
        if (!(V.call >= 0 && seen_pending == V.call - 1 && seen_call == V.call - 1)) return;
    } else {
        if (!((V.call < 0 || seen_call == V.call) && (V.redo == 2 || (seen_miss != 0) == (V.redo != 0)))) return;
    }
    if (do_fold) {
        DecideIn in;
        in.s_pred = s_pred;
        in.s_prior = 0.0;
        in.s_trial = s_trial;
        in.s_next = s_next;
        in.lam_in = lam_in;
        in.so = so_in;
        in.flags = fl_in;
        const DecideOut d = decide_finish(V, w, in, V.prev, 0, 0.0, nullptr, 0, red);
        if (!(d.accept && !(d.flags & (2u | 8u | 32u)))) return;
        fold_commit(V, w, d);
        if (!do_resolve && t == 0) {
            sc.pending = -1;
            sc.n_trials = 1;
            sc.done = 1;
        }
    } else if (do_resolve) {
        const double v = wave_sum(s_next);
        __syncthreads();
        if ((t & 63) == 0) red[0][t >> 6] = v;
        __syncthreads();
        if (t == 0) sc.sum_in[V.par] = ((red[0][0] + red[0][1]) + red[0][2]) + red[0][3];
    }
    if (!do_resolve) return;
    if (t == 0) over = 0u;
    __syncthreads();
    const int64_t count = 2 * V.m_total;
    unsigned long long prefix;
    long long rank;
    unsigned in_bin;
    select_resolve_loaded(hl, kSelBins, 11, 0ull, (count - 1) / 2, prefix, rank, lds_u, &in_bin);
    const unsigned bin = (unsigned)prefix;
    if ((unsigned)(t * 8) <= bin && bin < (unsigned)(t * 8 + 8)) {
        for (int q = 0; q < ranks; ++q)
            if (reinterpret_cast<const unsigned*>(gathered + (size_t)q * slot_len)[bin] > (unsigned)V.bucket_cap) over = 1u;
    }
    __syncthreads();
    const bool hit = lo != ~0ull && bin >= 1u && bin <= 2046u && in_bin <= 1024u && !over && !V.warm_force_miss;
    if (t == 0) {
        front_commit(V, w, hit, bin, rank, in_bin, false);
        if (hit) sc.sel_cnt = in_bin;
        if (V.wmax_ext) *V.wmax_ext = 0ull;
    }
    if (!hit) return;
    unsigned my_cnt = 0;
#pragma unroll
    for (int j = 0; j < 8; ++j) if ((unsigned)(t * 8 + j) == bin) my_cnt = mine[j];
    __syncthreads();
    if ((unsigned)(t * 8) <= bin && bin < (unsigned)(t * 8 + 8)) lds_u[20] = my_cnt;
    __syncthreads();
    const unsigned cnt = lds_u[20];
    const double* bucket = V.wbucket + (((size_t)w * 2 + V.par) * kSelBins + bin) * (size_t)V.bucket_cap;
    if (t == 0) bucket_out[0] = (double)cnt;
    for (unsigned q = t; q < cnt; q += 256) bucket_out[1 + q] = bucket[q];
}

__global__ void k_sh_clear_miss(DevView V) {
    V.sc[0].miss = 0;
    V.sc[0].fl[V.par] = 0u;
    V.host_head[0].flags = 0u;
}
void launch_sh_clear_miss(const DevView& V, hipStream_t s) { hipLaunchKernelGGL(k_sh_clear_miss, dim3(1), dim3(1), 0, s, V); }

void launch_sh_front(const DevView& V, const double* gathered, int ranks, int slot_len, double* bucket_out, int do_fold, int do_resolve, hipStream_t s) {
    hipLaunchKernelGGL(k_sh_front, dim3(1), dim3(256), 0, s, V, gathered, ranks, slot_len, bucket_out, do_fold, do_resolve);
}

__global__ __launch_bounds__(kObsBlock) void k_debug_project(DevView V, int w, double* est, double* J, double* wt) {
    const int m = V.m[w];
    const int k = blockIdx.x * kObsBlock + threadIdx.x;
    if (k >= m) return;
    const size_t ob = (size_t)w * V.obs_stride, mb = (size_t)w * V.m_max;
    const int pose = V.opose[2 * ob + k];
    const size_t pb = (size_t)w * V.n_max + pose;
    PoseCam pc;
    pose_camera(V.states_prev + pb * 10, V.intr + pb * 4, pc);
    double u, v, cam[3], d;
    project(pc, V.ox[ob + k], V.oy[ob + k], V.oz[ob + k], u, v, cam, d);
    est[2 * k] = u;
    est[2 * k + 1] = v;
    if (V.jac_f32) project_jacobian_f32(pc, cam, d, J + 12 * (size_t)k);
    else project_jacobian(pc, cam, d, J + 12 * (size_t)k);
    wt[k] = (V.wraw[mb + k] / bits_f64(V.sc[w].wmax_bits[V.par])) * V.oconf[ob + k];
}

__global__ __launch_bounds__(256) void k_broadcast_states(DevView V, int n, double lamda) {
    const int w = blockIdx.y;
    const double* src = V.states;
    double* dst = V.states + (size_t)w * V.n_max * 10;
    const int k = blockIdx.x * 256 + threadIdx.x;
    if (w > 0 && k < n * 10) dst[k] = src[k];
    if (k == 0) V.sc[w].lam[V.par] = lamda;
}

__global__ void k_set_counts(int* n_arr, int* m_arr, int w, int n, int m) {
    n_arr[w] = n;
    if (m >= 0) m_arr[w] = m;
}

__global__ void k_reset_calls(DevView V) {
    const int w = blockIdx.x * 64 + threadIdx.x;
    if (w < V.W) {
        V.sc[w].call_idx = 0;
        V.sc[w].pending = -1;
        V.sc[w].miss = 0;
    }
}

__global__ __launch_bounds__(1024) void k_clear_hist(DevView V, int which) {
    const int w = blockIdx.x;
    if (which == 2 && !V.sc[w].miss) return;
    unsigned* h0 = hist0_of(V, w, V.par);
    for (int b = threadIdx.x; b < kSelBins; b += 1024) h0[b] = 0u;
    if (which == 1) {
        unsigned* h12 = histd_of(V, w, 1);
        for (int b = threadIdx.x; b < 2 * kSelBins; b += 1024) h12[b] = 0u;
    }
}

void launch_clear_hist(const DevView& V, int which, hipStream_t s) {
    hipLaunchKernelGGL(k_clear_hist, dim3(V.W), dim3(1024), 0, s, V, which);
}

void launch_set_counts(const DevView& V, int w, int n, int m, hipStream_t s) {
    hipLaunchKernelGGL(k_set_counts, dim3(1), dim3(1), 0, s, const_cast<int*>(V.n), const_cast<int*>(V.m), w, n, m);
}

void launch_reset_calls(const DevView& V, hipStream_t s) {
    hipLaunchKernelGGL(k_reset_calls, dim3((V.W + 63) / 64), dim3(64), 0, s, V);
}

void launch_broadcast_states(const DevView& V, int n, double lamda, hipStream_t s) {
    hipLaunchKernelGGL(k_broadcast_states, dim3((n * 10 + 255) / 256, V.W), dim3(256), 0, s, V, n, lamda);
}


void launch_obs_residual(const DevView& V, double* abs_out, hipStream_t s) {
    if (abs_out) hipLaunchKernelGGL(k_obs_residual<false>, dim3(V.nblk_obs, V.W), dim3(kObsBlock), 0, s, V, abs_out);
    else hipLaunchKernelGGL(k_obs_residual<true>, dim3(V.nblk_obs, V.W), dim3(kObsBlock), 0, s, V, abs_out);
}

void launch_select(const DevView& V, bool with_digit0, hipStream_t s) {
    const int64_t count = V.abs_all ? V.abs_all_count : 2 * V.m_max;
    const dim3 b(256);
    if (!V.lat) {
        const int nb = (int)((count + 256 * 32 - 1) / (256 * 32));
        const dim3 g(nb > 0 ? nb : 1, V.W);
        if (with_digit0) hipLaunchKernelGGL((k_select_pass<0, false, 32>), g, b, 0, s, V);
        hipLaunchKernelGGL((k_select_pass<1, false, 32>), g, b, 0, s, V);
        hipLaunchKernelGGL((k_select_pass<2, true, 32>), g, b, 0, s, V);
    } else {
        const int nb = (int)((count + 256 * kSelItems - 1) / (256 * kSelItems));
        const dim3 g(nb > 0 ? nb : 1, V.W);
        if (with_digit0) hipLaunchKernelGGL((k_select_pass<0, false, kSelItems>), g, b, 0, s, V);
        hipLaunchKernelGGL((k_select_pass<1, false, kSelItems>), g, b, 0, s, V);
        hipLaunchKernelGGL((k_select_pass<2, true, kSelItems>), g, b, 0, s, V);
    }
}

void launch_select_warm(const DevView& V, hipStream_t s) {
    const int64_t count = 2 * V.m_max;
    if (!V.lat) {
#ifndef VBA_SELW_ITEMS
#define VBA_SELW_ITEMS 32
#endif
        const int nb = (int)((count + 256 * VBA_SELW_ITEMS - 1) / (256 * VBA_SELW_ITEMS));
        hipLaunchKernelGGL((k_select_warm<VBA_SELW_ITEMS>), dim3(nb > 0 ? nb : 1, V.W), dim3(256), 0, s, V);
    } else {
        const int nb = (int)((count + 256 * kSelItems - 1) / (256 * kSelItems));
        hipLaunchKernelGGL((k_select_warm<kSelItems>), dim3(nb > 0 ? nb : 1, V.W), dim3(256), 0, s, V);
    }
}

void launch_select_finish(const DevView& V, hipStream_t s) {
    hipLaunchKernelGGL(k_select_finish, dim3(V.W), dim3(256), 0, s, V);
}

#ifndef VBA_ACC_PAIR
#define VBA_ACC_PAIR 1
#endif
constexpr bool kPair = VBA_ACC_PAIR != 0;

template <bool F32>
static void launch_acc_batch(int G, dim3 g, dim3 b, hipStream_t s, const DevView& V) {
    if (G == 8) hipLaunchKernelGGL((k_obs_accumulate<8, kPair, true, F32>), g, b, 0, s, V);
    else hipLaunchKernelGGL((k_obs_accumulate<16, false, true, F32>), g, b, 0, s, V);
}

template <bool F32>
static void launch_acc_lanes(int G, dim3 g, dim3 b, hipStream_t s, const DevView& V) {
    switch (G) {
        case 4: hipLaunchKernelGGL((k_obs_accumulate<4, kPair, false, F32>), g, b, 0, s, V); break;
        case 8: hipLaunchKernelGGL((k_obs_accumulate<8, kPair, false, F32>), g, b, 0, s, V); break;
        case 16: hipLaunchKernelGGL((k_obs_accumulate<16, false, false, F32>), g, b, 0, s, V); break;
        case 32: hipLaunchKernelGGL((k_obs_accumulate<32, false, false, F32>), g, b, 0, s, V); break;
        default: hipLaunchKernelGGL((k_obs_accumulate<64, false, false, F32>), g, b, 0, s, V); break;
    }
}

void launch_obs_accumulate(const DevView& V, hipStream_t s) {
    const int G = V.acc_lanes;
    const int nb = (V.n_max * G + 255) / 256;
    const dim3 g(nb + (V.dyn_in_acc ? (V.n_max * kDynLanes + 255) / 256 : 0) + (V.sel_inline ? 1 : 0), V.W), b(256);
    if (V.median_ready && !V.dyn_in_acc && !V.sel_inline && (G == 8 || G == 16)) {
#ifndef VBA_ACC_GROUPS
#define VBA_ACC_GROUPS 4
#endif
        static const int groups_env = std::getenv("VBA_X_ACCGROUPS") ? std::atoi(std::getenv("VBA_X_ACCGROUPS")) : 0;
        int groups = VBA_ACC_GROUPS;
        while (groups > 1 && (int64_t)V.W * ((nb + groups - 1) / groups) < 2048) groups >>= 1;
        if (groups_env > 0) groups = groups_env;
        const dim3 gb((nb + groups - 1) / groups, V.W);
        if (V.jac_f32) launch_acc_batch<true>(G, gb, b, s, V);
        else launch_acc_batch<false>(G, gb, b, s, V);
        return;
    }
    if (V.jac_f32) launch_acc_lanes<true>(G, g, b, s, V);
    else launch_acc_lanes<false>(G, g, b, s, V);
    if (V.dyn_in_acc) launch_long_factor(V, s);
}

template <int EMIT>
static void launch_trial_emit(const DevView& V, hipStream_t s) {
    const dim3 g(V.nblk_obs + V.nblk_dyn, V.W), b(kObsBlock);
    const int f = V.fused_trial;
    if (f == 0 && !V.lat && !V.wbucket) {
        hipLaunchKernelGGL((k_trial<EMIT, 0, 2>), dim3(V.nblk_dyn, V.W), b, 0, s, V);
        hipLaunchKernelGGL((k_trial<EMIT, 0, 1>), dim3(V.nblk_obs, V.W), b, 0, s, V);
        return;
    }
    if (f == 1) hipLaunchKernelGGL((k_trial<EMIT, 1>), g, b, 0, s, V);
    else if (f == 2) hipLaunchKernelGGL((k_trial<EMIT, 2>), g, b, 0, s, V);
    else if (f == 3) hipLaunchKernelGGL((k_trial<EMIT, 3>), g, b, 0, s, V);
    else if (EMIT == 2 && V.trial_tiles == 8) hipLaunchKernelGGL((k_trial<EMIT, 0, 0, EMIT == 2 ? 8 : 1>), dim3((V.nblk_obs + 7) / 8 + V.nblk_dyn, V.W), b, 0, s, V);
    else if (EMIT == 2 && V.trial_tiles == 4) hipLaunchKernelGGL((k_trial<EMIT, 0, 0, EMIT == 2 ? 4 : 1>), dim3((V.nblk_obs + 3) / 4 + V.nblk_dyn, V.W), b, 0, s, V);
    else if (EMIT == 2 && V.trial_tiles == 2) hipLaunchKernelGGL((k_trial<EMIT, 0, 0, EMIT == 2 ? 2 : 1>), dim3((V.nblk_obs + 1) / 2 + V.nblk_dyn, V.W), b, 0, s, V);
    else hipLaunchKernelGGL((k_trial<EMIT, 0>), g, b, 0, s, V);
}

void launch_trial(const DevView& V, hipStream_t s) {
    if (V.emit == 2) launch_trial_emit<2>(V, s);
    else if (V.emit == 1) launch_trial_emit<1>(V, s);
    else launch_trial_emit<0>(V, s);
    launch_long_trial(V, s);
}

void launch_debug_project(const DevView& V, int w, int m, double* est, double* J, double* wt, hipStream_t s) {
    hipLaunchKernelGGL(k_debug_project, dim3((m + kObsBlock - 1) / kObsBlock), dim3(kObsBlock), 0, s, V, w, est, J, wt);
}

}
```

### vinsat_amd/csrc/vba_schedule.hip

```cpp
#include "vba_context.h"


void view_for_call(vba_handle h, DevView& V, const CallSpec& c) {
    V = h->V;
    V.m_total = 0; V.abs_all = nullptr; V.abs_all_count = 0;
    V.reg = h->reg ? 1 : 0;
    V.n_min = *std::min_element(h->n.begin(), h->n.end());
    V.call = c.call;
    V.par = c.par;
    V.states = h->S[c.par];
    V.wraw = h->wraw2 + (size_t)c.par * h->W * h->V.m_max;
    V.Hraw = h->Hraw2 + (size_t)c.par * h->W * h->n_max * 21;
    V.braw = h->braw2 + (size_t)c.par * h->W * h->n_max * 6;
    {
        const size_t wn = (size_t)c.par * h->W * h->n_max;
        V.xhat = h->dyn2[0] + wn * 6; V.Phi = h->dyn2[1] + wn * 36; V.rorb = h->dyn2[2] + wn * 6; V.fatt = h->dyn2[3] + wn;
        V.qgrad = h->dyn2[4] + wn * 3; V.Hd = h->dyn2[5] + wn * 9; V.Hu = h->dyn2[6] + wn * 9; V.Hl = h->dyn2[7] + wn * 9;
    }
    V.states_new = h->S[c.par ^ 1];
    V.states_prev = h->S[c.par];
    if (!c.host_out) V.host_states = nullptr;
    V.emit = c.emit;
    V.carry = c.carry;
    V.fold = c.fold ? 1 : 0;
    V.sel_inline = 0;
    V.median_ready = 0;
    V.redo = 0;
    V.pending_only = 0;
    V.warm_force_miss = h->warm_enabled == 2;
    V.pivot = h->pivot_mode;
    V.pack = 0;
    if (V.chunk <= 0 && !h->no_pack && h->W >= 2) {
        V.pack = 2;
        if (h->W >= h->pack_min) {
            V.pack = 1;
            for (int w = 1; w < h->W; ++w) if (h->n[w] != h->n[0]) V.pack = 2;
        }
    }
    fill_params(V.prm, c.iter, c.initialize);
    V.fused_trial = 0;
    if (V.lat && (h->fusion & 1)) {
        if (c.initialize) V.fused_trial = h->pivot_mode == 0 ? 1 : 3;
        else V.fused_trial = V.chunk > 0 ? 2 : 3;
        V.nblk_dyn = (V.n_max - 1 + 14) / 15;
    }
    V.fuse_blocks = (h->fusion & 2) ? 1 : 0;
    V.resident = !V.lat ? 0 : (h->fusion & 64) ? 2 : (h->fusion & 32) ? 1 : 0;
    V.chunk_waves = h->chunk_waves;
    V.asm_rows = (h->fusion & 8) ? 1 : 0;
    V.cr_levels = (h->fusion & 16) ? 1 : h->cr_levels;
    V.fuse_walk = ((h->fusion & 4) && !V.lat) ? 1 : 0;
}

int enqueue_front(vba_handle h, CallCtx& C, const CallSpec& c, bool exact_repeat, hipEvent_t* ev) {
    DevView& V = C.V;
    hipStream_t s = h->stream;
    auto mark = [&](int k) { if (ev && ev[k]) (void)hipEventRecord(ev[k], s); };
    const bool init = c.initialize != 0;
    V.sel_inline = 0;
    const bool ride = !init && !c.prof && V.lat;
    V.dyn_in_acc = ride ? 1 : 0;
    static const bool no_overlap = std::getenv("VBA_NO_OVERLAP") != nullptr;
    const bool overlap = !init && !c.prof && !ride && !no_overlap;
    auto fork_dynamics = [&]() -> int {
        HIPCHK(hipEventRecord(h->ev_fork, s));
        HIPCHK(hipStreamWaitEvent(h->aux_stream, h->ev_fork, 0));
        launch_dynamics(V, h->aux_stream);
        HIPCHK(hipEventRecord(h->ev_join, h->aux_stream));
        return VBA_OK;
    };
    const bool fork_late = overlap && c.fold;
    if (overlap && !fork_late) { if (int rc = fork_dynamics()) return rc; }
    mark(1);
    if (!c.carry) {
        launch_obs_residual(V, nullptr, s);
        mark(2);
        launch_select(V, false, s);
    } else if (c.carry == 2 && !exact_repeat) {
        mark(2);
        V.sel_inline = (V.wbucket && h->inline_select) ? 1 : 0;
        if (!V.sel_inline) launch_select_warm(V, s);
    } else if (c.carry == 1 && !exact_repeat) {
        mark(2);
        launch_select(V, false, s);
    } else {
        mark(2);
        launch_clear_hist(V, 2, s);
        launch_select(V, true, s);
    }
    if (fork_late) { if (int rc = fork_dynamics()) return rc; }
    V.median_ready = (!V.sel_inline && !V.lat) ? 1 : 0;
    if (V.median_ready) launch_select_finish(V, s);
    mark(3);
    launch_obs_accumulate(V, s);
    if (C.after_first && V.sel_inline) HIPCHK(hipEventRecord(C.after_first, s));
    mark(4);
    if (!init && !overlap && !ride) launch_dynamics(V, s);
    if (overlap) HIPCHK(hipStreamWaitEvent(s, h->ev_join, 0));
    mark(5);
    C.fuse_assemble = init && h->pivot_mode == 0 && V.fused_trial != 1;
    C.assembled = false;
    C.bands_ready = false;
    const bool need_bands = init ? V.fused_trial != 1 : !solve_forms_blocks(V);
    if (need_bands) {
        launch_assemble(V, C.fuse_assemble, s);
        C.assembled = true;
        C.bands_ready = !C.fuse_assemble;
    }
    mark(6);
    return VBA_OK;
}

void enqueue_trial(vba_handle h, CallCtx& C, const CallSpec& c, bool first, hipEvent_t ev_solve, int solve_redo) {
    DevView& V = C.V;
    hipStream_t s = h->stream;
    const bool init = c.initialize != 0;
    const int redo_all = V.redo;
    const bool pivoted_round = V.pivot != 0;
    const bool init_solve = init && (V.fused_trial == 1 ? pivoted_round : !(first && C.fuse_assemble));
    if (init_solve && !C.bands_ready) {
        launch_assemble(V, 0, s);
        C.assembled = C.bands_ready = true;
    }
    if (solve_redo >= 0) V.redo = solve_redo;
    if (init) {
        if (init_solve) launch_solve(V, 1, s);
    } else {
        launch_solve(V, 0, s);
    }
    V.redo = redo_all;
    if (ev_solve) (void)hipEventRecord(ev_solve, s);
    launch_trial(V, s);
}



int step_impl(vba_handle h, int iter, int initialize, float* prof, bool emit, int readback) {
    if (!h) return fail(VBA_EINVAL, "null handle");
    if (int rc_settle = settle(h)) return rc_settle;
    if (int rc = ready(h)) return rc;
    HIPCHK(hipSetDevice(h->device));
    hipStream_t s = h->stream;
    CallSpec c;
    c.iter = iter; c.initialize = initialize; c.call = -1; c.par = h->par;
    const int emit_kind = h->warm_enabled ? 2 : 1;
    c.emit = (h->carry_enabled && emit) ? emit_kind : 0;
    c.carry = h->carry_enabled ? h->carry_ok : 0;
    c.prof = prof != nullptr;
    h->carry_ok = 0;
    h->shc.carried = false;
    CallCtx C;
    view_for_call(h, C.V, c);
    DevView& V = C.V;
    if (h->need_hist_reset) {
        DevView Q = V;
        for (int p = 0; p < 2; ++p) { Q.par = p; launch_clear_hist(Q, 1, s); }
        h->need_hist_reset = false;
        h->hist_dirty = false;
    }
    if (!c.carry && h->hist_dirty) launch_clear_hist(V, 0, s);
    h->hist_dirty = c.emit != 0;
    struct ProfEvents {
        hipEvent_t e[VBA_NKERNELS + 1] = {};
        ~ProfEvents() { for (hipEvent_t q : e) if (q) (void)hipEventDestroy(q); }
    } pe;
    hipEvent_t* ev = pe.e;
    if (prof) {
        for (int k = 0; k <= VBA_NKERNELS; ++k) HIPCHK(hipEventCreate(&ev[k]));
    }
    auto mark = [&](int k) { if (prof) (void)hipEventRecord(ev[k], s); };
    struct Abandon {
        vba_handle h; bool armed = true;
        ~Abandon() { if (armed) { h->need_hist_reset = true; h->have_state.assign(h->W, 0); h->carry_ok = 0; } }
    } abandon{h};
    HIPCHK(hipEventRecord(h->ev0, s));
    mark(0);
    if (int rc = enqueue_front(h, C, c, false, prof ? ev : nullptr)) return rc;
    constexpr int kMaxTrials = 24;
    bool finished = false, first = true;
    int solve_redo = -1;
    for (int trial = 0; trial < kMaxTrials; ++trial) {
        enqueue_trial(h, C, c, first, (first && prof) ? ev[7] : nullptr, solve_redo);
        solve_redo = -1;
        if (first) mark(8);
        launch_decide(V, nullptr, 0, s);
        if (first) {
            mark(9);
            HIPCHK(hipEventRecord(h->ev1, s));
        }
        h->back_valid = false;
        if (readback >= 0) {
            HIPCHK(hipMemcpyAsync(h->h_back, V.states_new + (size_t)readback * h->n_max * 10, (size_t)h->n[readback] * 80, hipMemcpyDeviceToHost, s));
            HIPCHK(hipMemcpyAsync(h->h_back + (size_t)h->n_max * 10, V.sc + readback, sizeof(WinScalars), hipMemcpyDeviceToHost, s));
        }
        HIPCHK(hipGetLastError());
        if (int rc = read_heads(h)) return rc;
        first = false;
        bool all = true, repeat = false, miss = false;
        for (int w = 0; w < h->W; ++w) {
            all = all && head(h, w)->done;
            repeat = repeat || (head(h, w)->flags & 8u);
            miss = miss || (head(h, w)->flags & 32u);
        }
        if (miss) {
            for (int w = 0; w < h->W; ++w) if (head(h, w)->flags & 32u) h->h_head[w].flags = 0;
            h->warm_misses++;
            V.redo = 1;
            CallSpec cr = c;
            cr.prof = false;
            if (int rc = enqueue_front(h, C, cr, true, nullptr)) return rc;
            V.redo = 2;
            solve_redo = (c.initialize && C.fuse_assemble) ? 0 : 2;
            continue;
        }
        V.redo = 0;
        if (repeat && V.pivot == 0) {
            V.pivot = 2;
            h->fallbacks++;
            continue;
        }
        if (all) {
            h->back_valid = readback >= 0;
            finished = true;
            break;
        }
    }
    if (!finished)
        return fail(VBA_ESTATE, "LM loop did not terminate within " + std::to_string(kMaxTrials) + " trials (no outcome reported by the device)");
    abandon.armed = false;
    HIPCHK(hipEventElapsedTime(&h->last_ms, h->ev0, h->ev1));
    if (prof) {
        for (int k = 0; k < VBA_NKERNELS; ++k) {
            prof[k] = 0.f;
            (void)hipEventElapsedTime(&prof[k], ev[k], ev[k + 1]);
        }
        if (c.carry) prof[VBA_K_RESIDUAL] = 0.f;
        if (c.initialize && (C.fuse_assemble || V.fused_trial == 1)) prof[VBA_K_SOLVE] = 0.f;
        if (!C.assembled) prof[VBA_K_ASSEMBLE] = 0.f;
        if (c.initialize) prof[VBA_K_DYNAMICS] = 0.f;
    }
    h->par ^= 1;
    h->carry_ok = c.emit;
    h->stepped = true;
    h->last_pipelined = false;
    h->prev_res_iter = -1;
    h->last_iter = iter;
    h->last_init = initialize;
    return VBA_OK;
}

int vba_step(vba_handle h, int iter, int initialize) { return step_impl(h, iter, initialize, nullptr); }

static int finish_stalled_call(vba_handle h, const CallSpec& q, const std::vector<int>& stall_at, long& trials) {
    hipStream_t s = h->stream;
    const int sc_call = q.call;
    static const bool trace = std::getenv("VBA_TRACE") != nullptr;
    CallCtx C;
    view_for_call(h, C.V, q);
    DevView& V = C.V;
    C.fuse_assemble = q.initialize && h->pivot_mode == 0 && V.fused_trial != 1;
    C.assembled = q.initialize ? V.fused_trial != 1 : !solve_forms_blocks(V);
    C.bands_ready = C.assembled && !C.fuse_assemble;
    auto at_call = [&](int w) { return stall_at[w] == sc_call && head(h, w)->call_idx == sc_call; };
    bool any_miss = false;
    for (int w = 0; w < h->W; ++w) any_miss = any_miss || (at_call(w) && (head(h, w)->flags & 32u));
    V.pending_only = 1;
    launch_decide(V, nullptr, 0, s);
    V.pending_only = 0;
    if (any_miss) {
        for (int w = 0; w < h->W; ++w) if (at_call(w) && (head(h, w)->flags & 32u)) h->h_head[w].flags = 0;
        h->warm_misses++;
        V.redo = 1;
        if (int rc = enqueue_front(h, C, q, true, nullptr)) return rc;
        enqueue_trial(h, C, q, true);
        launch_decide(V, nullptr, 0, s);
        V.redo = 0;
        ++trials;
    }
    HIPCHK(hipGetLastError());
    if (int rc = read_heads(h)) return rc;
    bool finished = false;
    for (int trial = 0; trial <= 24; ++trial) {
        bool repeat = false, all = true;
        for (int w = 0; w < h->W; ++w) {
            if (!at_call(w)) continue;
            all = false;
            repeat = repeat || (head(h, w)->flags & 8u);
        }
        if (all) { finished = true; break; }
        if (trial == 24) break;
        if (repeat && V.pivot == 0) { V.pivot = 2; h->fallbacks++; }
        enqueue_trial(h, C, q, false);
        launch_decide(V, nullptr, 0, s);
        HIPCHK(hipGetLastError());
        if (int rc = read_heads(h)) return rc;
        ++trials;
        if (trace) {
            std::fprintf(stderr, "[vba]   call %d round %d pivot %d:", sc_call, trial, V.pivot);
            for (int w = 0; w < h->W && w < 8; ++w)
                std::fprintf(stderr, " w%d(call %d done %d flags %u ntr %d lam %g)", w, head(h, w)->call_idx, head(h, w)->done, head(h, w)->flags, head(h, w)->n_trials, head(h, w)->lamda);
            std::fprintf(stderr, "\n");
        }
    }
    if (!finished)
        return fail(VBA_ESTATE, "LM loop of call " + std::to_string(sc_call) + " did not terminate (no outcome reported by the device)");
    return VBA_OK;
}

int vba_run_schedule(vba_handle h, int ncalls, const int* iters, const int* inits, int* trials_total) {
    if (!h || !iters || !inits || ncalls < 1) return fail(VBA_EINVAL, "bad argument");
    if (int rc_settle = settle(h)) return rc_settle;
    if (int rc = ready(h)) return rc;
    HIPCHK(hipSetDevice(h->device));
    hipStream_t s = h->stream;
    const int par0 = h->par;
    const int emit_kind = h->carry_enabled ? (h->warm_enabled ? 2 : 1) : 0;
    const int carry0 = h->carry_enabled ? h->carry_ok : 0;
    h->carry_ok = 0;
    h->shc.carried = false;
    struct Abandon {
        vba_handle h; bool armed = true;
        ~Abandon() { if (armed) { h->need_hist_reset = true; h->have_state.assign(h->W, 0); h->carry_ok = 0; } }
    } abandon{h};
    auto spec = [&](int c, bool fold) {
        CallSpec q;
        q.iter = iters[c]; q.initialize = inits[c]; q.call = c; q.par = (par0 + c) & 1;
        q.carry = c == 0 ? carry0 : emit_kind;
        q.emit = emit_kind;
        q.fold = fold;
        return q;
    };
    {
        DevView V0;
        view_for_call(h, V0, spec(0, false));
        if (h->need_hist_reset) {
            DevView Q = V0;
            for (int p = 0; p < 2; ++p) { Q.par = p; launch_clear_hist(Q, 1, s); }
            h->need_hist_reset = false;
            h->hist_dirty = false;
        }
        if (!carry0 && h->hist_dirty) launch_clear_hist(V0, 0, s);
        launch_reset_calls(V0, s);
    }
    h->hist_dirty = emit_kind != 0;
    for (int w = 0; w < h->W; ++w) { h->h_head[w].call_idx = 0; h->h_head[w].done = 0; h->h_head[w].flags = 0; }
    long trials = 0;
    int next = 0;
    bool complete = false;
    const bool prof_pass = h->cprof.on;
    if (prof_pass) {
        while ((int)h->cprof.ev.size() < 4 * ncalls) {
            hipEvent_t e = nullptr;
            HIPCHK(hipEventCreate(&e));
            h->cprof.ev.push_back(e);
        }
    }
    static const bool no_graph = std::getenv("VBA_NO_GRAPH") != nullptr;
    for (int guard = 0; guard <= ncalls; ++guard) {
        bool capturing = false, replayed = false;
        std::vector<unsigned long long> gkey;
        std::vector<unsigned char> gviews;
        if (!no_graph && h->graph_enabled && guard == 0 && !prof_pass && h->V.lat && !h->graph_broken && next == 0 && (h->fusion & 96) == 0) {
            gkey.reserve(8 + 3 * (size_t)ncalls);
            gviews.resize((size_t)ncalls * sizeof(DevView));
            gkey.push_back((unsigned long long)ncalls); gkey.push_back((unsigned long long)par0); gkey.push_back((unsigned long long)carry0);
            gkey.push_back((unsigned long long)emit_kind); gkey.push_back((unsigned long long)h->pivot_mode);
            gkey.push_back((unsigned long long)h->inline_select | ((unsigned long long)h->fold_enabled << 1));
            gkey.push_back((unsigned long long)(uintptr_t)s);
            for (int c = 0; c < ncalls; ++c) {
                const bool fold = c > 0 && emit_kind == 2 && h->fold_enabled;
                DevView Vc;
                view_for_call(h, Vc, spec(c, fold));
                if (fold) fill_params(Vc.prev, iters[c - 1], inits[c - 1]);
                unsigned long long hsh = 1469598103934665603ull;
                const unsigned char* bytes = reinterpret_cast<const unsigned char*>(&Vc);
                std::memcpy(gviews.data() + (size_t)c * sizeof(DevView), bytes, sizeof(DevView));
                for (size_t o = 0; o + 8 <= sizeof(DevView); o += 8) {
                    unsigned long long wd;
                    std::memcpy(&wd, bytes + o, 8);
                    hsh = (hsh ^ wd) * 1099511628211ull;
                    hsh ^= hsh >> 29;
                }
                gkey.push_back(hsh); gkey.push_back((unsigned long long)iters[c]); gkey.push_back((unsigned long long)inits[c]);
            }
            size_t hit = h->graphs.size();
            for (size_t k = 0; k < h->graphs.size(); ++k)
                if (h->graphs[k].key == gkey && h->graphs[k].views == gviews) { hit = k; break; }
            if (hit < h->graphs.size()) {
                if (hit != 0) std::rotate(h->graphs.begin(), h->graphs.begin() + hit, h->graphs.begin() + hit + 1);
                if (hipGraphLaunch(h->graphs[0].exec, s) == hipSuccess) { replayed = true; h->graph_replays++; }
                else { (void)hipGetLastError(); h->graph_broken = true; }
            } else {
                if (hipStreamBeginCapture(s, hipStreamCaptureModeRelaxed) == hipSuccess) capturing = true;
                else { (void)hipGetLastError(); h->graph_broken = true; }
            }
        }
        struct CaptureGuard {
            hipStream_t s; bool* on;
            ~CaptureGuard() {
                if (*on) {
                    hipGraph_t g = nullptr;
                    (void)hipStreamEndCapture(s, &g);
                    if (g) (void)hipGraphDestroy(g);
                    (void)hipGetLastError();
                }
            }
        } capture_guard{s, &capturing};
        auto enqueue_pass = [&]() -> int {
        for (int c = next; c < ncalls && !replayed; ++c) {
            const bool fold = c > next && emit_kind == 2 && h->fold_enabled;
            const CallSpec q = spec(c, fold);
            CallCtx C;
            view_for_call(h, C.V, q);
            if (fold) fill_params(C.V.prev, iters[c - 1], inits[c - 1]);
            hipEvent_t marks[VBA_NKERNELS + 1] = {};
            hipEvent_t* pe = nullptr;
            if (prof_pass && guard == 0) {
                pe = h->cprof.ev.data() + (size_t)4 * c;
                marks[1] = pe[0];
                marks[6] = pe[1];
            }
            if (int rc = enqueue_front(h, C, q, false, pe ? marks : nullptr)) return rc;
            enqueue_trial(h, C, q, true, pe ? pe[2] : nullptr);
            if (pe) HIPCHK(hipEventRecord(pe[3], s));
            const bool next_folds = c + 1 < ncalls && emit_kind == 2 && h->fold_enabled;
            if (!next_folds) launch_decide(C.V, nullptr, 0, s);
        }
        return VBA_OK;
        };
        if (int rc = enqueue_pass()) return rc;
        if (capturing) {
            static const int inject = std::getenv("VBA_GRAPH_FAIL_INJECT") ? std::atoi(std::getenv("VBA_GRAPH_FAIL_INJECT")) : 0;
            hipGraph_t g = nullptr;
            capturing = false;
            hipGraphExec_t exec = nullptr;
            bool ok = hipStreamEndCapture(s, &g) == hipSuccess && g != nullptr && inject != 1;
            if (ok) ok = hipGraphInstantiate(&exec, g, nullptr, nullptr, 0) == hipSuccess && inject != 2;
            if (g) (void)hipGraphDestroy(g);
            if (ok && (inject == 3 || hipGraphLaunch(exec, s) != hipSuccess)) ok = false;
            if (!ok) {
                (void)hipGetLastError();
                if (exec) (void)hipGraphExecDestroy(exec);
                h->graph_broken = true;
                if (int rc = enqueue_pass()) return rc;
            } else {
            constexpr size_t kGraphCache = 8;
            if (h->graphs.size() >= kGraphCache) {
                HIPCHK(hipStreamSynchronize(s));
                (void)hipGraphExecDestroy(h->graphs.back().exec);
                h->graphs.pop_back();
            }
            vba_context::GraphEntry ge;
            ge.key = gkey;
            ge.views = std::move(gviews);
            ge.exec = exec;
            h->graphs.insert(h->graphs.begin(), std::move(ge));
            h->graph_captures++;
            }
        }
        HIPCHK(hipGetLastError());
        if (int rc = read_heads(h)) return rc;
        trials += (long)(ncalls - next);
        std::vector<int> stalled, stall_at((size_t)h->W);
        for (int w = 0; w < h->W; ++w) {
            const int c = (int)head(h, w)->call_idx;
            stall_at[w] = c;
            if (c < ncalls && std::find(stalled.begin(), stalled.end(), c) == stalled.end()) stalled.push_back(c);
        }
        if (prof_pass && guard == 0 && stalled.empty()) {
            for (int c = 0; c < ncalls; ++c) {
                const hipEvent_t* pe = h->cprof.ev.data() + (size_t)4 * c;
                for (int k = 0; k < 3; ++k) {
                    float ms = 0.f;
                    if (k == 1 && inits[c]) continue;
                    if (hipEventElapsedTime(&ms, pe[k], pe[k + 1]) == hipSuccess) {
                        h->cprof.ms[k] += ms;
                        h->cprof.launches[k]++;
                    }
                }
            }
        }
        if (stalled.empty()) { complete = true; break; }
        std::sort(stalled.begin(), stalled.end());
        static const bool trace = std::getenv("VBA_TRACE") != nullptr;
        if (trace) {
            std::fprintf(stderr, "[vba] pass from call %d:", next);
            for (int w = 0; w < h->W && w < 8; ++w)
                std::fprintf(stderr, " w%d(call %d done %d flags %u ntr %d)", w, head(h, w)->call_idx, head(h, w)->done, head(h, w)->flags, head(h, w)->n_trials);
            std::fprintf(stderr, "\n");
        }
        for (int sc_call : stalled) {
            if (int rc = finish_stalled_call(h, spec(sc_call, false), stall_at, trials)) return rc;
        }
        next = stalled.front() + 1;
        if (next >= ncalls) { complete = true; break; }
    }
    if (!complete) {
        complete = true;
        for (int w = 0; w < h->W; ++w) complete = complete && head(h, w)->call_idx >= ncalls;
        if (!complete) return fail(VBA_ESTATE, "chained schedule did not complete (a window never reached its last call)");
    }
    abandon.armed = false;
    if (trials_total) *trials_total = (int)trials;
    h->par = (par0 + ncalls) & 1;
    h->carry_ok = emit_kind;
    h->stepped = true;
    h->last_pipelined = false;
    h->last_iter = iters[ncalls - 1];
    h->last_init = inits[ncalls - 1];
    return VBA_OK;
}


int vba_set_schedule_graph(vba_handle h, int on) {
    if (!h) return fail(VBA_EINVAL, "null handle");
    if (int rc = settle(h)) return rc;
    h->graph_enabled = on != 0;
    return VBA_OK;
}

int vba_schedule_graph_stats(vba_handle h, int* captures, int* replays) {
    if (!h) return fail(VBA_EINVAL, "null handle");
    if (captures) *captures = (int)h->graph_captures;
    if (replays) *replays = (int)h->graph_replays;
    return VBA_OK;
}

int vba_set_chain_profile(vba_handle h, int on) {
    if (!h) return fail(VBA_EINVAL, "null handle");
    if (int rc = settle(h)) return rc;
    h->cprof.on = on != 0;
    return VBA_OK;
}



int vba_chain_profile(vba_handle h, double* ms, int64_t* launches, int reset) {
    if (!h) return fail(VBA_EINVAL, "null handle");
    for (int k = 0; k < 3; ++k) {
        if (ms) ms[k] = h->cprof.ms[k];
        if (launches) launches[k] = h->cprof.launches[k];
        if (reset) { h->cprof.ms[k] = 0.0; h->cprof.launches[k] = 0; }
    }
    return VBA_OK;
}


int vba_step_profiled(vba_handle h, int iter, int initialize, float* ms) {
    if (!ms) return fail(VBA_EINVAL, "null ms");
    return step_impl(h, iter, initialize, ms);
}

static int take_back(vba_handle h, double* states_out, double* lamda_out, double* last_hessian, int* n_trials, unsigned* flags) {
    if (h->back_valid) {
        const WinScalars* sc = reinterpret_cast<const WinScalars*>(h->h_back + (size_t)h->n_max * 10);
        if (states_out) std::memcpy(states_out, h->h_back, (size_t)h->n[0] * 80);
        unpack_scalars(sc, h->par, lamda_out, last_hessian, n_trials, flags);
        return VBA_OK;
    }
    return vba_get_states(h, 0, states_out, lamda_out, last_hessian, n_trials, flags);
}

int vba_iterate(vba_handle h, int iter, int initialize, double lamda_in, const double* states_in, double* states_out,
                double* lamda_out, double* last_hessian, int* n_trials, unsigned* flags) {
    if (int rc = vba_set_states(h, 0, states_in, lamda_in)) return rc;
    if (int rc = step_impl(h, iter, initialize, nullptr, false, 0)) return rc;
    return take_back(h, states_out, lamda_out, last_hessian, n_trials, flags);
}

static bool can_pipeline(vba_handle h);
static bool host_watch_changed(vba_handle h);
static int iterate_pipelined(vba_handle h, int iter, int initialize, double* states_out, double* lamda_out, double* last_hessian,
                             int* n_trials, unsigned* flags);

int vba_iterate_open(vba_handle h, int iter, int initialize, double lamda_in, const double* states_in, double* states_out,
                     double* lamda_out, double* last_hessian, int* n_trials, unsigned* flags) {
    if (int rc = vba_set_states(h, 0, states_in, lamda_in)) return rc;
    if (can_pipeline(h)) return iterate_pipelined(h, iter, initialize, states_out, lamda_out, last_hessian, n_trials, flags);
    const bool watch_changed = host_watch_changed(h);
    if (int rc = step_impl(h, iter, initialize, nullptr, false, 0)) return rc;
    if (int rc = take_back(h, states_out, lamda_out, last_hessian, n_trials, flags)) return rc;
    if (flags && watch_changed) *flags |= VBA_FLAG_HOST_CHANGED;
    return VBA_OK;
}

static bool host_watch_changed(vba_handle h) {
    for (const auto& w : h->watch)
        if (w.live && std::memcmp(w.live, w.copy, w.bytes) != 0) return true;
    return false;
}
static size_t host_watch_bytes(vba_handle h) {
    size_t b = 0;
    for (const auto& w : h->watch) if (w.live) b += w.bytes;
    return b;
}
static bool watch_begin(vba_handle h) {
    if (host_watch_bytes(h) < 65536) return false;
    auto& W = h->ww;
    if (W.started && W.owner != getpid()) return false;
    if (!W.started) {
        W.started = true;
        W.owner = getpid();
        W.th = std::thread([h]() {
            auto& Q = h->ww;
            unsigned long long taken = 0;
            for (;;) {
                {
                    std::unique_lock<std::mutex> lk(Q.m);
                    Q.cv.wait(lk, [&] { return Q.quit || Q.seq != taken; });
                    if (Q.quit) return;
                    taken = Q.seq;
                }
                Q.changed = host_watch_changed(h);
                Q.done_seq.store(taken, std::memory_order_release);
            }
        });
    }
    {
        std::lock_guard<std::mutex> lk(W.m);
        ++W.seq;
    }
    W.cv.notify_one();
    return true;
}
static bool watch_end(vba_handle h, bool begun) {
    if (!begun) return host_watch_changed(h);
    auto& W = h->ww;
    const auto t0 = std::chrono::steady_clock::now();
    const unsigned long long mine = W.seq;
    for (unsigned spins = 0; W.done_seq.load(std::memory_order_acquire) != mine; ++spins) {
        __builtin_ia32_pause();
        if ((spins & 1023u) == 1023u && std::chrono::steady_clock::now() - t0 > std::chrono::milliseconds(20)) return host_watch_changed(h);
    }
    return W.changed;
}
void watch_quiesce(vba_handle h) {
    auto& W = h->ww;
    if (!W.started || W.owner != getpid()) return;
    while (W.done_seq.load(std::memory_order_acquire) != W.seq) std::this_thread::yield();
}
void watch_stop(vba_handle h) {
    auto& W = h->ww;
    if (!W.started) return;
    if (W.owner != getpid()) {
        W.th.detach();
        W.started = false;
        return;
    }
    {
        std::lock_guard<std::mutex> lk(W.m);
        W.quit = true;
    }
    W.cv.notify_one();
    W.th.join();
    W.started = false;
}

static bool can_pipeline(vba_handle h) {
    return h->pipeline && h->W == 1 && h->h_states_map && h->carry_enabled && h->warm_enabled >= 1 && h->fold_enabled && h->inline_select &&
           h->V.wbucket != nullptr && h->pivot_mode == 0 && h->V.chunk > 0 && h->V.lat;
}

static int iterate_pipelined(vba_handle h, int iter, int initialize, double* states_out, double* lamda_out, double* last_hessian,
                             int* n_trials, unsigned* flags) {
    if (int rc = ready(h)) return rc;
    HIPCHK(hipSetDevice(h->device));
    hipStream_t s = h->stream;
    constexpr int emit_kind = 2;
    initialize = initialize ? 1 : 0;
    if (h->prev_res_iter >= 0) {
        h->pred_iter[h->prev_res_iter & 63] = iter;
        h->pred_init[h->prev_res_iter & 63] = initialize;
    }
    bool consumed = false;
    if (h->spec.valid) {
        if (h->spec.iter == iter && h->spec.init == initialize && h->spec.reg == h->reg) {
            consumed = true;
            h->spec_hits++;
        } else if (int rc = settle(h)) {
            return rc;
        }
    }
    struct Abandon {
        vba_handle h; bool armed = true;
        ~Abandon() { if (armed) { h->need_hist_reset = true; h->have_state.assign(h->W, 0); h->carry_ok = 0; h->spec.valid = false; h->prev_res_iter = -1; } }
    } abandon{h};
    auto call_spec = [&](int c, int it, int in, int carry, bool fold) {
        CallSpec q;
        q.iter = it; q.initialize = in; q.call = c; q.par = (h->chain_par0 + c) & 1;
        q.carry = carry; q.emit = emit_kind; q.fold = fold;
        q.host_out = true;
        return q;
    };
    bool watch_changed = false;
    int c;
    if (consumed) {
        c = h->spec.c;
        h->spec.valid = false;
    } else {
        const int carry0 = h->carry_ok;
        h->carry_ok = 0;
        h->shc.carried = false;
        h->chain_par0 = h->par;
        c = 0;
        const CallSpec q = call_spec(0, iter, initialize, carry0, false);
        CallCtx C;
        view_for_call(h, C.V, q);
        if (h->need_hist_reset) {
            DevView Q = C.V;
            for (int p = 0; p < 2; ++p) { Q.par = p; launch_clear_hist(Q, 1, s); }
            h->need_hist_reset = false;
            h->hist_dirty = false;
        }
        if (!carry0 && h->hist_dirty) launch_clear_hist(C.V, 0, s);
        launch_reset_calls(C.V, s);
        h->h_head[0].call_idx = 0; h->h_head[0].done = 0; h->h_head[0].flags = 0;
        if (int rc = enqueue_front(h, C, q, false, nullptr)) return rc;
        enqueue_trial(h, C, q, true);
    }
    h->hist_dirty = true;
    int ni = h->pred_iter[iter & 63], nin = h->pred_init[iter & 63];
    if (ni == -1) { ni = iter + 1; nin = initialize; }
    const bool speculate = ni >= 0;
    const CallSpec qc = call_spec(c, iter, initialize, emit_kind, false);
    const int par_c = qc.par;
    const bool watching = watch_begin(h);
    struct WatchJoin {
        vba_handle h; bool begun; bool joined = false;
        bool end() { joined = true; return watch_end(h, begun); }
        ~WatchJoin() { if (begun && !joined) (void)watch_end(h, true); }
    } wj{h, watching};
    if (speculate) {
        const CallSpec qn = call_spec(c + 1, ni, nin, emit_kind, true);
        CallCtx C;
        view_for_call(h, C.V, qn);
        fill_params(C.V.prev, iter, initialize);
        C.after_first = h->ev_first;
        if (int rc = enqueue_front(h, C, qn, false, nullptr)) return rc;
        enqueue_trial(h, C, qn, true);
        HIPCHK(hipGetLastError());
        HIPCHK(hipEventSynchronize(h->ev_first));
        watch_changed = wj.end();
    } else {
        CallCtx C;
        view_for_call(h, C.V, qc);
        launch_decide(C.V, nullptr, 0, s);
        HIPCHK(hipGetLastError());
        HIPCHK(hipStreamSynchronize(s));
        watch_changed = wj.end();
    }
    h->stepped = true;
    h->last_pipelined = true;
    h->last_iter = iter;
    h->last_init = initialize;
    h->back_valid = false;
    const bool clean = (int)head(h, 0)->call_idx >= c + 1;
    if (clean) {
        h->par = par_c ^ 1;
        const volatile WinHead* hd = head(h, 0);
        if (states_out) std::memcpy(states_out, h->h_states_map + (size_t)par_c * h->n_max * 10, (size_t)h->n[0] * 80);
        if (lamda_out) *lamda_out = hd->lamda;
        if (last_hessian) for (int k = 0; k < 81; ++k) last_hessian[k] = hd->last_hessian[k];
        if (n_trials) *n_trials = 1;
        if (flags) *flags = (hd->flags & 7u) | (watch_changed ? VBA_FLAG_HOST_CHANGED : 0u);
        if (speculate) {
            h->spec.valid = true; h->spec.iter = ni; h->spec.init = nin; h->spec.reg = h->reg; h->spec.c = c + 1;
            h->carry_ok = 0;
        } else {
            h->carry_ok = emit_kind;
        }
        h->prev_res_iter = iter;
        abandon.armed = false;
        return VBA_OK;
    }
    HIPCHK(hipStreamSynchronize(s));
    {
        std::vector<int> stall_at(1, c);
        long trials = 0;
        if ((int)head(h, 0)->call_idx != c) return fail(VBA_ESTATE, "pipelined call: the window is at call " + std::to_string(head(h, 0)->call_idx) + ", expected " + std::to_string(c));
        if (int rc = finish_stalled_call(h, qc, stall_at, trials)) return rc;
    }
    h->par = par_c ^ 1;
    h->carry_ok = emit_kind;
    h->prev_res_iter = iter;
    abandon.armed = false;
    if (int rc = vba_get_states(h, 0, states_out, lamda_out, last_hessian, n_trials, flags)) return rc;
    if (flags && watch_changed) *flags |= VBA_FLAG_HOST_CHANGED;
    return VBA_OK;
}

int vba_iterate_resident(vba_handle h, int iter, int initialize, double* states_out, double* lamda_out, double* last_hessian,
                         int* n_trials, unsigned* flags) {
    if (!h) return fail(VBA_EINVAL, "null handle");
    if (!h->stepped) return fail(VBA_ESTATE, "vba_iterate_resident follows a call that left its result on the device");
    if (can_pipeline(h)) return iterate_pipelined(h, iter, initialize, states_out, lamda_out, last_hessian, n_trials, flags);
    const bool watch_changed = host_watch_changed(h);
    if (int rc = step_impl(h, iter, initialize, nullptr, true, 0)) return rc;
    if (int rc = take_back(h, states_out, lamda_out, last_hessian, n_trials, flags)) return rc;
    if (flags && watch_changed) *flags |= VBA_FLAG_HOST_CHANGED;
    return VBA_OK;
}
```

### vinsat_amd/csrc/vba_sharded_api.hip

```cpp
#include "vba_context.h"

int64_t vba_sh_partial_count(int n) { return 27 * (int64_t)n + 2; }

static void sharded_view(vba_handle h, DevView& V) {
    CallSpec c;
    c.iter = h->last_iter; c.initialize = h->last_init; c.call = -1; c.par = h->par;
    view_for_call(h, V, c);
    V.fuse_walk = 0;
    V.m_total = h->V.m_total;
}

int vba_sh_stage1(vba_handle h, int iter, int initialize, int64_t m_total, double* d_abs_local) {
    if (!h || !d_abs_local || m_total < 1) return fail(VBA_EINVAL, "bad argument");
    if (int rc_settle = settle(h)) return rc_settle;
    if (h->W != 1) return fail(VBA_EINVAL, "sharded mode uses a single window per handle");
    if (h->reg) return fail(VBA_EINVAL, "sharded mode does not take a prior (vba_set_prior)");
    if (int rc = ready(h)) return rc;
    HIPCHK(hipSetDevice(h->device));
    hipStream_t s = h->stream;
    h->V.m_total = m_total;
    h->sharded = true;
    h->last_iter = iter;
    h->last_init = initialize;
    h->carry_ok = false;
    h->shc.carried = false;
    DevView V;
    sharded_view(h, V);
    if (h->hist_dirty || h->need_hist_reset) {
        DevView Q = V;
        for (int p = 0; p < 2; ++p) { Q.par = p; launch_clear_hist(Q, 1, s); }
        h->hist_dirty = h->need_hist_reset = false;
    }
    launch_obs_residual(V, d_abs_local, s);
    HIPCHK(hipGetLastError());
    return VBA_OK;
}

int vba_sh_stage2(vba_handle h, const double* d_abs_all, int64_t count_all, double* d_partial_local) {
    if (!h || !d_abs_all || !d_partial_local || count_all < 1) return fail(VBA_EINVAL, "bad argument");
    if (h->V.m_total < 1 || count_all < 2 * h->V.m_total) return fail(VBA_ESTATE, "stage1 has not run or count_all < 2*m_total");
    HIPCHK(hipSetDevice(h->device));
    hipStream_t s = h->stream;
    DevView V;
    sharded_view(h, V);
    V.abs_all = d_abs_all;
    V.abs_all_count = count_all;
    launch_select(V, true, s);
    h->sh_rode = !h->last_init && V.lat;
    V.dyn_in_acc = h->sh_rode ? 1 : 0;
    launch_obs_accumulate(V, s);
    launch_shard_pack(V, d_partial_local, s);
    HIPCHK(hipGetLastError());
    return VBA_OK;
}

int vba_sh_stage3(vba_handle h, const double* d_partial_all, int ranks, double* d_trial_local) {
    if (!h || !d_trial_local) return fail(VBA_EINVAL, "bad argument");
    if (h->V.m_total < 1) return fail(VBA_ESTATE, "stage1 has not run");
    HIPCHK(hipSetDevice(h->device));
    hipStream_t s = h->stream;
    CallSpec c;
    c.iter = h->last_iter; c.initialize = h->last_init; c.call = -1; c.par = h->par;
    CallCtx C;
    sharded_view(h, C.V);
    DevView& V = C.V;
    const bool init = h->last_init != 0;
    if (d_partial_all) {
        if (ranks < 1) return fail(VBA_EINVAL, "ranks must be >= 1");
        launch_shard_reduce(V, d_partial_all, ranks, s);
        if (!init && !h->sh_rode) launch_dynamics(V, s);
        const bool need_bands = init ? V.fused_trial != 1 : !solve_forms_blocks(V);
        if (need_bands) launch_assemble(V, 0, s);
        h->sh_bands_ready = need_bands;
        h->sh_pivot = h->pivot_mode;
    }
    V.pivot = h->sh_pivot;
    C.fuse_assemble = false;
    C.assembled = C.bands_ready = h->sh_bands_ready;
    enqueue_trial(h, C, c, d_partial_all != nullptr);
    h->sh_bands_ready = C.bands_ready;
    launch_shard_trial_sum(V, d_trial_local, s);
    HIPCHK(hipGetLastError());
    return VBA_OK;
}

int vba_sh_stage4(vba_handle h, const double* d_trial_all, int ranks, int* done) {
    if (!h || !d_trial_all || !done || ranks < 1) return fail(VBA_EINVAL, "bad argument");
    HIPCHK(hipSetDevice(h->device));
    DevView V;
    sharded_view(h, V);
    launch_decide(V, d_trial_all, ranks, h->stream);
    HIPCHK(hipGetLastError());
    if (int rc = read_heads(h)) return rc;
    *done = head(h, 0)->done;
    if (!*done && (head(h, 0)->flags & 8u) && h->sh_pivot == 0) {
        h->sh_pivot = 2;
        h->fallbacks++;
    }
    if (*done) {
        h->stepped = true;
        h->V.m_total = 0;
        h->par ^= 1;
    }
    return VBA_OK;
}

namespace {
void* open_rccl(const char* path) {
    void* dl = dlopen(path, RTLD_NOW | RTLD_NOLOAD);
    if (!dl) dl = dlopen(path, RTLD_NOW | RTLD_LOCAL);
    return dl;
}
}

int vba_sh_unique_id(const char* rccl_path, void* id128) {
    if (!rccl_path || !id128) return fail(VBA_EINVAL, "null argument");
    void* dl = open_rccl(rccl_path);
    if (!dl) return fail(VBA_EINVAL, std::string("cannot open ") + rccl_path + ": " + dlerror());
    auto get_id = reinterpret_cast<ncclResult_t (*)(ncclUniqueId*)>(dlsym(dl, "ncclGetUniqueId"));
    if (!get_id) { dlclose(dl); return fail(VBA_EINVAL, "ncclGetUniqueId not found in the named library"); }
    ncclUniqueId id;
    const ncclResult_t rc = get_id(&id);
    dlclose(dl);
    if (rc != ncclSuccess) return fail(VBA_EHIP, "ncclGetUniqueId failed (" + std::to_string((int)rc) + ")");
    static_assert(sizeof(id) == 128, "unique id size");
    std::memcpy(id128, &id, sizeof(id));
    return VBA_OK;
}

int vba_sh_comm_init(vba_handle h, const char* rccl_path, const void* id128, int nranks, int rank) {
    if (!h || !rccl_path || !id128 || nranks < 1 || rank < 0 || rank >= nranks) return fail(VBA_EINVAL, "bad argument");
    if (int rc_settle = settle(h)) return rc_settle;
    if (h->W != 1) return fail(VBA_EINVAL, "sharded mode uses a single window per handle");
    if (h->shc.comm) return fail(VBA_ESTATE, "the handle has a communicator already");
    h->sharded = true;
    HIPCHK(hipSetDevice(h->device));
    auto& S = h->shc;
    S.dl = open_rccl(rccl_path);
    if (!S.dl) return fail(VBA_EINVAL, std::string("cannot open ") + rccl_path + ": " + dlerror());
    auto init_rank = reinterpret_cast<ncclResult_t (*)(ncclComm_t*, int, ncclUniqueId, int)>(dlsym(S.dl, "ncclCommInitRank"));
    S.all_gather = reinterpret_cast<decltype(S.all_gather)>(dlsym(S.dl, "ncclAllGather"));
    S.comm_destroy = reinterpret_cast<decltype(S.comm_destroy)>(dlsym(S.dl, "ncclCommDestroy"));
    S.error_string = reinterpret_cast<decltype(S.error_string)>(dlsym(S.dl, "ncclGetErrorString"));
    if (!init_rank || !S.all_gather || !S.comm_destroy || !S.error_string) {
        dlclose(S.dl);
        S = {};
        return fail(VBA_EINVAL, "the named library does not export the RCCL entry points");
    }
    ncclUniqueId id;
    std::memcpy(&id, id128, sizeof(id));
    const ncclResult_t rc = init_rank(&S.comm, nranks, id, rank);
    if (rc != ncclSuccess) {
        const std::string why = S.error_string(rc);
        dlclose(S.dl);
        S = {};
        return fail(VBA_EHIP, "ncclCommInitRank failed: " + why);
    }
    S.nranks = nranks;
    S.rank = rank;
    return VBA_OK;
}

int vba_sh_comm_destroy(vba_handle h) {
    if (!h) return VBA_OK;
    auto& S = h->shc;
    if (!S.comm && !S.buf) return VBA_OK;
    hipSetDevice(h->device);
    hipStreamSynchronize(h->stream);
    if (S.comm) S.comm_destroy(S.comm);
    if (S.buf) hipFree(S.buf);
    if (S.buf2) hipFree(S.buf2);
    if (S.dl) dlclose(S.dl);
    S = {};
    return VBA_OK;
}

namespace {

int sh_ensure_buffers(vba_handle h, int64_t m_total) {
    auto& S = h->shc;
    const int n = h->n[0];
    const int64_t m_pad = (m_total + S.nranks - 1) / S.nranks;
    if (h->m[0] > m_pad) return fail(VBA_EINVAL, "this rank holds more rows than ceil(m_total / ranks)");
    const int64_t pc = vba_sh_partial_count(n);
    const int64_t R = S.nranks;
    if (S.m_total != m_total || S.n != n) {
        HIPCHK(hipStreamSynchronize(h->stream));
        if (S.buf) { HIPCHK(hipFree(S.buf)); S.buf = nullptr; }
        const int64_t total = 2 * m_pad * (1 + R) + pc * (1 + R) + 2 * (1 + R) + 64;
        HIPCHK(hipMalloc((void**)&S.buf, (size_t)total * 8));
        S.abs_local = S.buf;
        S.abs_all = S.abs_local + 2 * m_pad;
        S.partial_local = S.abs_all + 2 * m_pad * R;
        S.partial_all = S.partial_local + pc;
        S.trial_local = S.partial_all + pc * R;
        S.trial_all = S.trial_local + 2;
        S.m_total = m_total; S.m_pad = m_pad; S.n = n;
        S.m_local = -1;
        S.carried = false;
    }
    if (S.m_local != h->m[0]) {
        HIPCHK(hipStreamSynchronize(h->stream));
        std::vector<double> inf((size_t)(2 * m_pad), INFINITY);
        HIPCHK(hipMemcpy(S.abs_local, inf.data(), inf.size() * 8, hipMemcpyHostToDevice));
        S.m_local = h->m[0];
        S.carried = false;
    }
    if (S.protocol == 1) {
        const int64_t keys = 2 * m_total;
        const int shift = keys <= 300000 ? 44 : (keys <= 600000 ? 43 : 42);
        if (h->V.warm_shift != shift) {
            h->V.warm_shift = shift;
            h->carry_ok = 0;
            S.carried = false;
        }
    }
    const int nbo = h->V.nblk_obs, cap = h->V.bucket_cap;
    const int lenA = (1024 + nbo + h->V.trial_stride + 3) & ~3, lenB = (cap + 1 + 3) & ~3;
    if (S.protocol == 1 && cap > 0 && (S.lenA != lenA || S.lenB != lenB || !S.buf2)) {
        HIPCHK(hipStreamSynchronize(h->stream));
        if (S.buf2) { HIPCHK(hipFree(S.buf2)); S.buf2 = nullptr; }
        const size_t total = (size_t)lenA * (2 + R) + (size_t)lenB * (1 + R) + 64;
        HIPCHK(hipMalloc((void**)&S.buf2, total * 8));
        HIPCHK(hipMemset(S.buf2, 0, total * 8));
        HIPCHK(hipStreamSynchronize(nullptr));
        S.sendA[0] = S.buf2;
        S.sendA[1] = S.sendA[0] + lenA;
        S.recvA = S.sendA[1] + lenA;
        S.sendB = S.recvA + (size_t)lenA * R;
        S.recvB = S.sendB + lenB;
        S.lenA = lenA; S.lenB = lenB;
        S.carried = false;
    }
    return VBA_OK;
}

int sh_gather(vba_handle h, const double* src, double* dst, int64_t count) {
    auto& S = h->shc;
    const ncclResult_t rc = S.all_gather(src, dst, (size_t)count, ncclDouble, S.comm, h->stream);
    if (rc != ncclSuccess) return fail(VBA_EHIP, std::string("ncclAllGather failed: ") + S.error_string(rc));
    return VBA_OK;
}

int sh_call_classic(vba_handle h, int iter, int initialize, int64_t m_total, int* n_trials) {
    auto& S = h->shc;
    const int n = h->n[0];
    const int64_t pc = vba_sh_partial_count(n);
    if (int rc = vba_sh_stage1(h, iter, initialize, m_total, S.abs_local)) return rc;
    if (int rc = sh_gather(h, S.abs_local, S.abs_all, 2 * S.m_pad)) return rc;
    if (int rc = vba_sh_stage2(h, S.abs_all, 2 * S.m_pad * S.nranks, S.partial_local)) return rc;
    if (int rc = sh_gather(h, S.partial_local, S.partial_all, pc)) return rc;
    int trials = 0;
    for (bool first = true;; first = false) {
        if (int rc = vba_sh_stage3(h, first ? S.partial_all : nullptr, S.nranks, S.trial_local)) return rc;
        if (int rc = sh_gather(h, S.trial_local, S.trial_all, 2)) return rc;
        int done = 0;
        if (int rc = vba_sh_stage4(h, S.trial_all, S.nranks, &done)) return rc;
        ++trials;
        if (done) break;
        if (trials >= 24) return fail(VBA_ESTATE, "sharded BA call: the LM loop did not terminate within 24 trials");
    }
    if (n_trials) *n_trials = trials;
    return VBA_OK;
}

struct Sh2 {
    vba_handle h;
    int R;
    const int *iters, *inits;
    int ncalls, par0;

    CallSpec spec(int c, bool carried, bool fold) const {
        CallSpec q;
        q.iter = iters[c]; q.initialize = inits[c]; q.call = c; q.par = (par0 + c) & 1;
        q.carry = carried ? 2 : 0;
        q.emit = 2;
        q.fold = fold;
        return q;
    }
    void view(DevView& V, const CallSpec& q) const {
        auto& S = h->shc;
        view_for_call(h, V, q);
        V.fuse_walk = 0;
        V.m_total = S.m_total;
        V.hist0_ext[0] = reinterpret_cast<unsigned*>(S.sendA[0]);
        V.hist0_ext[1] = reinterpret_cast<unsigned*>(S.sendA[1]);
        V.part_next = S.sendA[q.par ^ 1] + 1024;
        V.part_trial = V.part_next + V.nblk_obs;
        V.sel_inline = 0;
        V.pivot = h->sh_pivot;
    }

    int enqueue_call(int c, bool carried, bool fold) {
        auto& S = h->shc;
        hipStream_t s = h->stream;
        const CallSpec q = spec(c, carried, fold);
        const int n = h->n[0];
        const int64_t pc = vba_sh_partial_count(n);
        const bool init = q.initialize != 0;
        CallCtx C;
        view(C.V, q);
        DevView& V = C.V;
        h->sh_pivot = h->pivot_mode;
        V.pivot = h->sh_pivot;
        V.dyn_in_acc = (!init && V.lat) ? 1 : 0;
        if (carried) {
            if (fold) fill_params(V.prev, iters[c - 1], inits[c - 1]);
            if (R > 1) V.wmax_ext = reinterpret_cast<unsigned long long*>(S.partial_local + (size_t)27 * n);
            launch_sh_front(V, S.recvA, R, S.lenA, S.sendB, fold ? 1 : 0, 1, s);
            if (int rc = sh_gather(h, S.sendB, S.recvB, S.lenB)) return rc;
            DevView Va = V;
            Va.sel_slots = S.recvB; Va.sel_nslots = R; Va.sel_slot_stride = S.lenB;
            Va.Hraw = S.partial_local; Va.braw = S.partial_local + (size_t)21 * n;
            launch_obs_accumulate(Va, s);
            if (int rc = sh_gather(h, S.partial_local, S.partial_all, pc)) return rc;
            if (R > 1) launch_shard_reduce(V, S.partial_all, R, s, 0);
            else { V.Hraw = S.partial_all; V.braw = S.partial_all + (size_t)21 * n; }
        } else {
            DevView Q = V;
            for (int p = 0; p < 2; ++p) { Q.par = p; launch_clear_hist(Q, 1, s); }
            V.redo = 2;
            launch_sh_clear_miss(V, s);
            launch_obs_residual(V, S.abs_local, s);
            if (int rc = sh_gather(h, S.abs_local, S.abs_all, 2 * S.m_pad)) return rc;
            DevView Vs = V;
            Vs.abs_all = S.abs_all; Vs.abs_all_count = 2 * S.m_pad * R;
            launch_select(Vs, true, s);
            launch_obs_accumulate(Vs, s);
            launch_shard_pack(V, S.partial_local, s);
            if (int rc = sh_gather(h, S.partial_local, S.partial_all, pc)) return rc;
            launch_shard_reduce(V, S.partial_all, R, s, 1);
        }
        if (!init && !V.dyn_in_acc) launch_dynamics(V, s);
        const bool need_bands = init ? V.fused_trial != 1 : !solve_forms_blocks(V);
        if (need_bands) launch_assemble(V, 0, s);
        C.fuse_assemble = false;
        C.assembled = C.bands_ready = need_bands;
        enqueue_trial(h, C, q, true);
        if (int rc = sh_gather(h, S.sendA[q.par ^ 1], S.recvA, S.lenA)) return rc;
        return VBA_OK;
    }

    int finish_stalled(int c, bool carried, long& trials) {
        auto& S = h->shc;
        hipStream_t s = h->stream;
        const CallSpec q = spec(c, carried, false);
        CallCtx C;
        view(C.V, q);
        DevView& V = C.V;
        const int n = h->n[0];
        if (R == 1 && carried) { V.Hraw = S.partial_all; V.braw = S.partial_all + (size_t)21 * n; }
        V.redo = 2;
        const bool init = q.initialize != 0;
        C.fuse_assemble = false;
        C.assembled = C.bands_ready = init ? V.fused_trial != 1 : !solve_forms_blocks(V);
        for (int round = 0; round <= 24; ++round) {
            launch_shard_trial_sum(V, S.trial_local, s);
            if (int rc = sh_gather(h, S.trial_local, S.trial_all, 2)) return rc;
            launch_decide(V, S.trial_all, R, s);
            HIPCHK(hipGetLastError());
            if (int rc = read_heads(h)) return rc;
            if (head(h, 0)->done) {
                if (int rc = sh_gather(h, S.sendA[q.par ^ 1], S.recvA, S.lenA)) return rc;
                S.fallbacks_lm++;
                return VBA_OK;
            }
            if (round == 24) break;
            if ((head(h, 0)->flags & 8u) && h->sh_pivot == 0) { h->sh_pivot = 2; h->fallbacks++; }
            V.pivot = h->sh_pivot;
            enqueue_trial(h, C, q, false);
            ++trials;
        }
        return fail(VBA_ESTATE, "sharded BA call: the LM loop did not terminate within 24 rounds");
    }
};

}

int vba_sh_set_protocol(vba_handle h, int carried_keys) {
    if (!h) return fail(VBA_EINVAL, "null handle");
    if (int rc = settle(h)) return rc;
    h->shc.protocol = carried_keys ? 1 : 0;
    h->shc.carried = false;
    return VBA_OK;
}

int vba_sh_stats(vba_handle h, int64_t* bytes_first_exchange, int64_t* fallbacks_miss, int64_t* fallbacks_lm) {
    if (!h) return fail(VBA_EINVAL, "null handle");
    auto& S = h->shc;
    if (bytes_first_exchange) *bytes_first_exchange = (S.protocol == 1 && S.lenA && h->m_max == S.m_pad) ? (int64_t)S.lenA * 8 : 16 * S.m_pad;
    if (fallbacks_miss) *fallbacks_miss = S.fallbacks_miss;
    if (fallbacks_lm) *fallbacks_lm = S.fallbacks_lm;
    return VBA_OK;
}

int vba_sh_run_schedule(vba_handle h, int ncalls, const int* iters, const int* inits, int64_t m_total, int* trials_total) {
    if (!h || !iters || !inits || ncalls < 1 || m_total < 1) return fail(VBA_EINVAL, "bad argument");
    auto& S = h->shc;
    if (!S.comm) return fail(VBA_ESTATE, "vba_sh_comm_init has not run");
    if (int rc_settle = settle(h)) return rc_settle;
    if (h->W != 1) return fail(VBA_EINVAL, "sharded mode uses a single window per handle");
    if (h->reg) return fail(VBA_EINVAL, "sharded mode does not take a prior (vba_set_prior)");
    if (int rc = ready(h)) return rc;
    HIPCHK(hipSetDevice(h->device));
    if (int rc = sh_ensure_buffers(h, m_total)) return rc;
    if (h->fusion_auto && S.protocol != 0 && !(h->fusion & 1)) h->fusion = 15;
    if (S.protocol == 0 || !h->V.wbucket || !h->V.lat || !(h->fusion & 1) || h->V.chunk <= 0 || h->m_max != S.m_pad) {
        long total = 0;
        for (int c = 0; c < ncalls; ++c) {
            int t = 0;
            if (int rc = sh_call_classic(h, iters[c], inits[c], m_total, &t)) return rc;
            total += t;
        }
        S.carried = false;
        if (trials_total) *trials_total = (int)total;
        return VBA_OK;
    }
    hipStream_t s = h->stream;
    h->V.m_total = m_total;
    Sh2 P{h, S.nranks, iters, inits, ncalls, h->par};
    bool carried0 = S.carried && h->carry_ok == 2 && S.carried_par == h->par;
    h->carry_ok = 0;
    S.carried = false;
    struct Abandon {
        vba_handle h; bool armed = true;
        ~Abandon() { if (armed) { h->need_hist_reset = true; h->have_state.assign(h->W, 0); h->carry_ok = 0; h->V.m_total = 0; } }
    } abandon{h};
    {
        DevView V0;
        P.view(V0, P.spec(0, false, false));
        launch_reset_calls(V0, s);
    }
    h->h_head[0].call_idx = 0; h->h_head[0].done = 0; h->h_head[0].flags = 0;
    long trials = 0;
    int next = 0;
    bool first_carried = carried0;
    for (int guard = 0; guard <= 2 * ncalls + 2; ++guard) {
        for (int c = next; c < ncalls; ++c) {
            const bool carried = c == next ? first_carried : true;
            const bool fold = carried && c > next;
            if (int rc = P.enqueue_call(c, carried, fold)) return rc;
        }
        {
            CallSpec q = P.spec(ncalls - 1, true, true);
            q.call = ncalls; q.par = (P.par0 + ncalls) & 1;
            DevView V;
            P.view(V, q);
            fill_params(V.prev, iters[ncalls - 1], inits[ncalls - 1]);
            launch_sh_front(V, S.recvA, P.R, S.lenA, S.sendB, 1, 0, s);
        }
        HIPCHK(hipGetLastError());
        if (int rc = read_heads(h)) return rc;
        const int at = (int)head(h, 0)->call_idx;
        if (at >= ncalls) { trials += (long)(ncalls - next); break; }
        if (head(h, 0)->flags & 32u) {
            trials += (long)(at - next);
            S.fallbacks_miss++;
            h->warm_misses++;
            h->h_head[0].flags = 0;
            next = at;
            first_carried = false;
            continue;
        }
        trials += (long)(at - next + 1);
        if (int rc = P.finish_stalled(at, at == next ? first_carried : true, trials)) return rc;
        next = at + 1;
        first_carried = true;
        if (next >= ncalls) break;
    }
    if ((int)head(h, 0)->call_idx < ncalls) return fail(VBA_ESTATE, "sharded schedule did not complete (the window never reached its last call)");
    abandon.armed = false;
    h->par = (P.par0 + ncalls) & 1;
    h->carry_ok = 2;
    S.carried = true;
    S.carried_par = h->par;
    h->V.m_total = 0;
    h->stepped = true;
    h->last_pipelined = false;
    h->last_iter = iters[ncalls - 1];
    h->last_init = inits[ncalls - 1];
    if (trials_total) *trials_total = (int)trials;
    return VBA_OK;
}

int vba_sh_call(vba_handle h, int iter, int initialize, int64_t m_total, int* n_trials) {
    return vba_sh_run_schedule(h, 1, &iter, &initialize, m_total, n_trials);
}
```

Measured before the change: 23200 BA iterations/s.

## Defer state upload into graph via mapped staging and cache graph lookups by identity

vba_set_states for a single window now copies states into mapped coherent host memory and defers the upload. The first kernel of the schedule (k_reset_calls, now captured in the graph) reads the staged states directly and also clears the histogram. This removes separate H2D memcpy and clear launches per call. A generation counter bumped by every setter lets graph lookup match on a cheap identity vector before building per-call DevView keys and hashing them, cutting host work per replay. It adds staleness risk if some state change misses touch(), and entry timing stamps are added under a compile flag.

```diff
diff --git a/vinsat_amd/csrc/vba_api.hip b/vinsat_amd/csrc/vba_api.hip
--- a/vinsat_amd/csrc/vba_api.hip
+++ b/vinsat_amd/csrc/vba_api.hip
@@ -1,6 +1,9 @@
 #include "vba_context.h"
 
 thread_local std::string g_err;
+#ifdef VBA_ENTRY_STAMPS
+EntryStamps g_estamps;
+#endif
 
 int fail(int code, const std::string& msg) {
     g_err = msg;
@@ -33,6 +36,7 @@
 
 int read_heads(vba_handle h) {
     HIPCHK(hipStreamSynchronize(h->stream));
+    VBA_ESTAMP(0);
     for (int w = 0; w < h->W; ++w)
         if (h->h_head[w].flags & 64u)
             return fail(VBA_ESTATE, "resident solve: a block of window " + std::to_string(w) + " timed out waiting for its producers (vba_set_fusion bits 5, 6)");
@@ -56,8 +60,21 @@
     return hipStreamCreateWithPriority(s, hipStreamNonBlocking, want > 0 ? greatest : least);
 }
 
-int settle(vba_handle h, bool boundary) {
+int flush_states(vba_handle h) {
+    if (!h->pend.on) return VBA_OK;
+    h->pend.on = false;
+    HIPCHK(hipSetDevice(h->device));
+    const size_t n10 = (size_t)h->pend.n * 10;
+    HIPCHK(hipMemcpyAsync(h->S[h->pend.par], h->h_stage_map, n10 * 8, hipMemcpyHostToDevice, h->stream));
+    HIPCHK(hipMemcpyAsync(&h->V.sc[0].lam[h->pend.par], h->h_stage_map + n10, 8, hipMemcpyHostToDevice, h->stream));
+    HIPCHK(hipEventRecord(h->ev_stage, h->stream));
+    h->stage_copy = true;
+    return VBA_OK;
+}
+
+int settle(vba_handle h, bool boundary, bool keep_staged) {
     if (!h) return VBA_OK;
+    if (!keep_staged) { if (int rc = flush_states(h)) return rc; }
     if (!h->spec.valid) {
         if (boundary) h->prev_res_iter = -1;
         return VBA_OK;
@@ -267,6 +284,8 @@
     if ((windows == 1 && (hipEventCreateWithFlags(&h->ev_first, hipEventDisableTiming) != hipSuccess ||
                           hipHostMalloc((void**)&h->h_states_map, (size_t)2 * n_max * 10 * sizeof(double), hipHostMallocMapped | hipHostMallocCoherent) != hipSuccess ||
                           hipHostGetDevicePointer((void**)&h->V.host_states, h->h_states_map, 0) != hipSuccess)) ||
+        (windows == 1 && lat && (hipHostMalloc((void**)&h->h_stage_map, ((size_t)n_max * 10 + 2) * sizeof(double), hipHostMallocMapped | hipHostMallocCoherent) != hipSuccess ||
+                                 hipHostGetDevicePointer((void**)&h->d_stage_map, h->h_stage_map, 0) != hipSuccess)) ||
         hipStreamCreateWithFlags(&h->own_stream, hipStreamNonBlocking) != hipSuccess ||
         (!lat && create_aux_stream(&h->aux_stream) != hipSuccess) ||
         hipEventCreate(&h->ev0) != hipSuccess || hipEventCreate(&h->ev1) != hipSuccess ||
@@ -318,6 +337,7 @@
 
 int vba_destroy(vba_handle h) {
     if (!h) return VBA_OK;
+    h->pend.on = false;
     (void)settle(h);
     watch_stop(h);
     hipSetDevice(h->device);
@@ -328,6 +348,7 @@
     for (auto& ge : h->graphs) if (ge.exec) (void)hipGraphExecDestroy(ge.exec);
     if (h->ev_first) hipEventDestroy(h->ev_first);
     if (h->h_states_map) hipHostFree(h->h_states_map);
+    if (h->h_stage_map) hipHostFree(h->h_stage_map);
     if (h->ev_fork) hipEventDestroy(h->ev_fork);
     if (h->ev_join) hipEventDestroy(h->ev_join);
     if (h->ev0) hipEventDestroy(h->ev0);
@@ -354,6 +375,7 @@
 int vba_set_solver2(vba_handle h, int chunk, int chunk2) {
     if (!h) return fail(VBA_EINVAL, "null handle");
     if (int rc_settle = settle(h)) return rc_settle;
+    h->touch();
     if (chunk < 2 || chunk > 60 || (chunk2 != 0 && chunk2 != -1 && (chunk2 < 2 || chunk2 > 60)))
         return fail(VBA_EINVAL, "chunk sizes must be in [2, 60] (chunk2 = 0: single level, -1: cyclic reduction)");
     if (chunk2 == -1 && (h->n_max + chunk - 1) / chunk - 1 > 128)
@@ -367,6 +389,7 @@
 int vba_set_solver(vba_handle h, int chunk) {
     if (!h) return fail(VBA_EINVAL, "null handle");
     if (int rc_settle = settle(h)) return rc_settle;
+    h->touch();
     h->V.chunk2 = 0;
     if (chunk == -1) {
         h->no_pack = 0;
@@ -413,6 +436,7 @@
 int vba_set_integrator(vba_handle h, int hop100) {
     if (!h) return fail(VBA_EINVAL, "null handle");
     if (int rc_settle = settle(h)) return rc_settle;
+    h->touch();
     h->V.hop = hop100 ? 1 : 0;
     h->V.nblk_long = h->V.hop ? 0 : *std::max_element(h->n_long.begin(), h->n_long.end());
     return VBA_OK;
@@ -421,6 +445,7 @@
 static int vba_set_accumulate_lanes(vba_handle h, int lanes) {
     if (!h) return fail(VBA_EINVAL, "null handle");
     if (int rc_settle = settle(h)) return rc_settle;
+    h->touch();
     if (lanes == 0) {
         const double avg = (double)h->m_max / (double)h->n_max;
         int G = 4;
@@ -436,6 +461,7 @@
 static int vba_set_trial_tiles(vba_handle h, int tiles) {
     if (!h) return fail(VBA_EINVAL, "null handle");
     if (int rc_settle = settle(h)) return rc_settle;
+    h->touch();
     if (tiles == 0) {
         const int64_t blocks = (int64_t)h->W * h->V.nblk_obs;
         tiles = blocks >= 600 ? 4 : (blocks >= 150 ? 2 : 1);
@@ -448,6 +474,7 @@
 static int vba_set_key_carry(vba_handle h, int on) {
     if (!h) return fail(VBA_EINVAL, "null handle");
     if (int rc_settle = settle(h)) return rc_settle;
+    h->touch();
     h->carry_enabled = on != 0;
     h->carry_ok = false;
     return VBA_OK;
@@ -456,6 +483,7 @@
 static int vba_set_fusion(vba_handle h, int mask) {
     if (!h) return fail(VBA_EINVAL, "null handle");
     if (int rc_settle = settle(h)) return rc_settle;
+    h->touch();
     if (mask < 0 || mask > 127) return fail(VBA_EINVAL, "mask must be in [0, 127]");
 #ifndef VBA_VARIANTS
     if (mask & (16 | 32 | 64)) return fail(VBA_EINVAL, "mask bits 4 .. 6 select comparison variants that this build does not carry (make VARIANTS=1)");
@@ -468,6 +496,7 @@
 static int vba_set_chunk_waves(vba_handle h, int waves) {
     if (!h) return fail(VBA_EINVAL, "null handle");
     if (int rc_settle = settle(h)) return rc_settle;
+    h->touch();
     if (waves != 1 && waves != 2) return fail(VBA_EINVAL, "waves must be 1 or 2");
     h->chunk_waves = waves;
     return VBA_OK;
@@ -476,6 +505,7 @@
 static int vba_set_warm_select(vba_handle h, int on) {
     if (!h) return fail(VBA_EINVAL, "null handle");
     if (int rc_settle = settle(h)) return rc_settle;
+    h->touch();
     h->warm_enabled = on == 2 ? 2 : (on != 0);
     h->inline_select = on != 3;
     return VBA_OK;
@@ -484,6 +514,7 @@
 static int vba_set_warm_shift(vba_handle h, int shift) {
     if (!h) return fail(VBA_EINVAL, "null handle");
     if (int rc_settle = settle(h)) return rc_settle;
+    h->touch();
     if (shift < 42 || shift > 51) return fail(VBA_EINVAL, "shift must be in [42, 51]");
     h->V.warm_shift = shift;
     h->carry_ok = 0;
@@ -493,6 +524,7 @@
 static int vba_set_bucket_cap(vba_handle h, int cap) {
     if (!h) return fail(VBA_EINVAL, "null handle");
     if (int rc_settle = settle(h)) return rc_settle;
+    h->touch();
     if (!h->bucket_cap_alloc) return fail(VBA_ESTATE, "this handle has no bin buckets (16 windows or more)");
     if (cap != 0 && (cap < 8 || cap > h->bucket_cap_alloc)) return fail(VBA_EINVAL, "cap must be 0 (default) or in [8, allocated capacity]");
     h->V.bucket_cap = cap ? cap : h->bucket_cap_alloc;
@@ -513,6 +545,7 @@
 static int vba_set_pipeline(vba_handle h, int on) {
     if (!h) return fail(VBA_EINVAL, "null handle");
     if (int rc = settle(h)) return rc;
+    h->touch();
     h->pipeline = on != 0;
     return VBA_OK;
 }
@@ -533,6 +566,7 @@
 static int vba_set_jacobian_f32(vba_handle h, int on) {
     if (!h) return fail(VBA_EINVAL, "null handle");
     if (int rc_settle = settle(h)) return rc_settle;
+    h->touch();
     if (on != 0 && on != 1) return fail(VBA_EINVAL, "jacobian_f32 must be 0 (fp64, default) or 1 (fp32)");
     h->V.jac_f32 = on;
     return VBA_OK;
@@ -541,6 +575,7 @@
 static int vba_set_pivoting(vba_handle h, int always) {
     if (!h) return fail(VBA_EINVAL, "null handle");
     if (int rc_settle = settle(h)) return rc_settle;
+    h->touch();
     h->pivot_mode = always ? 1 : 0;
     return VBA_OK;
 }
@@ -554,6 +589,7 @@
 int vba_set_stream(vba_handle h, void* hip_stream, int external) {
     if (!h) return fail(VBA_EINVAL, "null handle");
     if (int rc_settle = settle(h)) return rc_settle;
+    h->touch();
     hipStreamSynchronize(h->stream);
     h->stream = external ? (hipStream_t)hip_stream : h->own_stream;
     return VBA_OK;
@@ -563,6 +599,7 @@
                             const double* conf, const int64_t* ii) {
     if (int rc = check_window(h, window)) return rc;
     if (int rc_settle = settle(h, true)) return rc_settle;
+    h->touch();
     if (!xyz || !uv || !conf || !ii) return fail(VBA_EINVAL, "null observation array");
     h->carry_ok = false;
     if (n < 2 || n > h->n_max) return fail(VBA_EINVAL, "n out of range (need 2 <= n <= n_max)");
@@ -615,6 +652,7 @@
                       const int64_t* time_idx) {
     if (int rc = check_window(h, window)) return rc;
     if (int rc_settle = settle(h, true)) return rc_settle;
+    h->touch();
     if (!intrinsics || !cumrot_last || !time_idx) return fail(VBA_EINVAL, "null pose-constant array");
     h->carry_ok = false;
     if (n < 2 || n > h->n_max) return fail(VBA_EINVAL, "n out of range (need 2 <= n <= n_max)");
@@ -675,6 +713,7 @@
 int vba_upload_prior(vba_handle h, int window, int n, const double* states_prior, const double* hessian_state) {
     if (int rc = check_window(h, window)) return rc;
     if (int rc_settle = settle(h, true)) return rc_settle;
+    h->touch();
     if (!states_prior || !hessian_state) return fail(VBA_EINVAL, "null prior array");
     if (!h->have_obs[window] && !h->have_win[window]) return fail(VBA_ESTATE, "upload the window before its prior");
     if (n != h->n[window]) return fail(VBA_EINVAL, "the prior needs one row per pose of the window");
@@ -696,15 +735,29 @@
 int vba_set_prior(vba_handle h, int on) {
     if (!h) return fail(VBA_EINVAL, "null handle");
     h->reg = on != 0;
+    h->touch();
     return VBA_OK;
 }
 
 int vba_set_states(vba_handle h, int window, const double* states, double lamda) {
     if (!h) return fail(VBA_EINVAL, "null handle");
-    if (int rc_settle = settle(h, true)) return rc_settle;
+    VBA_ESTAMP(1);
+    if (int rc_settle = settle(h, true, true)) return rc_settle;
     if (!states) return fail(VBA_EINVAL, "null states");
     h->carry_ok = 0;
     double* S = h->S[h->par];
+    if (h->h_stage_map && window == 0 && (h->have_obs[0] || h->have_win[0])) {
+        if (h->stage_kernel) { HIPCHK(hipSetDevice(h->device)); HIPCHK(hipStreamSynchronize(h->stream)); h->stage_kernel = false; }
+        if (h->stage_copy) { HIPCHK(hipEventSynchronize(h->ev_stage)); h->stage_copy = false; }
+        const int n = h->n[0];
+        std::memcpy(h->h_stage_map, states, (size_t)n * 80);
+        h->h_stage_map[(size_t)n * 10] = lamda;
+        h->pend.on = true; h->pend.par = h->par; h->pend.n = n;
+        h->have_state[0] = 1;
+        VBA_ESTAMP(2);
+        return VBA_OK;
+    }
+    if (int rc = flush_states(h)) return rc;
     if (window == -1) {
         const int n = h->n[0];
         for (int w = 0; w < h->W; ++w) {
@@ -735,6 +788,7 @@
     HIPCHK(hipMemcpyAsync(&h->V.sc[window].lam[h->par], h->h_stage + (size_t)h->n_max * 10, 8, hipMemcpyHostToDevice, h->stream));
     HIPCHK(hipEventRecord(h->ev_stage, h->stream));
     h->have_state[window] = 1;
+    VBA_ESTAMP(2);
     return VBA_OK;
 }
 
@@ -854,6 +908,15 @@
     double wmax;
     std::memcpy(&wmax, &sc.wmax_bits[V.par], 8);
     switch (what) {
+#ifdef VBA_ENTRY_STAMPS
+        case 103: {
+            if (capacity < 12) return fail(VBA_EINVAL, "debug buffer too small");
+            for (int k = 0; k < 6; ++k) { out[2 * k] = g_estamps.cnt[k]; out[2 * k + 1] = g_estamps.sum[k]; }
+            g_estamps = EntryStamps();
+            *count = 12;
+            return VBA_OK;
+        }
+#endif
 #ifdef VBA_RESIDENT_STAMPS
         case 100:
             return copy(V.cR2 + (size_t)window * V.res_stride * 4, (int64_t)V.res_stride * 4);
diff --git a/vinsat_amd/csrc/vba_context.h b/vinsat_amd/csrc/vba_context.h
--- a/vinsat_amd/csrc/vba_context.h
+++ b/vinsat_amd/csrc/vba_context.h
@@ -33,6 +33,21 @@
         if (e_ != hipSuccess)                                                                          \
             return fail(VBA_EHIP, std::string(#expr) + ": " + hipGetErrorString(e_));                  \
     } while (0)
+
+#ifdef VBA_ENTRY_STAMPS
+struct EntryStamps { int last = -1; double t_last = 0.0; double sum[6] = {}; double cnt[6] = {}; };
+extern EntryStamps g_estamps;
+inline void entry_stamp(int k) {
+    const double now = std::chrono::duration<double, std::nano>(std::chrono::steady_clock::now().time_since_epoch()).count();
+    EntryStamps& E = g_estamps;
+    if (E.last == (k + 5) % 6) { E.sum[k] += now - E.t_last; E.cnt[k] += 1.0; }
+    E.last = k;
+    E.t_last = now;
+}
+#define VBA_ESTAMP(k) entry_stamp(k)
+#else
+#define VBA_ESTAMP(k) ((void)0)
+#endif
 
 struct Arena {
     char* base = nullptr;
@@ -81,6 +96,11 @@
     int par = 0;
     bool need_hist_reset = false;
     hipEvent_t ev_stage = nullptr;
+    double* h_stage_map = nullptr;
+    const double* d_stage_map = nullptr;
+    struct PendingStates { bool on = false; int par = 0, n = 0; } pend;
+    bool stage_copy = false;
+    bool stage_kernel = false;
     std::vector<int> n, m;
     std::vector<char> have_obs, have_win, have_state, have_prior;
     bool reg = false;
@@ -127,8 +147,11 @@
     int cr_levels = 2;
     int fusion = 15;
     bool fusion_auto = true;
-    struct GraphEntry { std::vector<unsigned long long> key; std::vector<unsigned char> views; hipGraphExec_t exec = nullptr; };
+    struct GraphEntry { std::vector<unsigned long long> key, ident; std::vector<unsigned char> views; hipGraphExec_t exec = nullptr; };
     std::vector<GraphEntry> graphs;
+    std::vector<unsigned long long> ident_now;
+    unsigned long long gen = 0;
+    void touch() { ++gen; }
     bool graph_broken = false;
     bool graph_enabled = true;
     long graph_replays = 0, graph_captures = 0;
@@ -176,7 +199,8 @@
 int read_heads(vba_handle h);
 const volatile WinHead* head(vba_handle h, int w);
 hipError_t create_aux_stream(hipStream_t* s);
-int settle(vba_handle h, bool boundary = false);
+int settle(vba_handle h, bool boundary = false, bool keep_staged = false);
+int flush_states(vba_handle h);
 int ready(vba_handle h);
 void unpack_scalars(const WinScalars* sc, int par, double* lamda, double* last_hessian, int* n_trials, unsigned* flags);
 
diff --git a/vinsat_amd/csrc/vba_launch.h b/vinsat_amd/csrc/vba_launch.h
--- a/vinsat_amd/csrc/vba_launch.h
+++ b/vinsat_amd/csrc/vba_launch.h
@@ -12,7 +12,7 @@
 void launch_obs_accumulate(const DevView& V, hipStream_t s);
 void launch_trial(const DevView& V, hipStream_t s);
 void launch_clear_hist(const DevView& V, int which, hipStream_t s);
-void launch_reset_calls(const DevView& V, hipStream_t s);
+void launch_reset_calls(const DevView& V, hipStream_t s, const double* stage = nullptr, int n10 = 0, int clear0 = 0);
 void launch_set_counts(const DevView& V, int w, int n, int m, hipStream_t s);
 void launch_broadcast_states(const DevView& V, int n, double lamda, hipStream_t s);
 void launch_debug_project(const DevView& V, int w, int m, double* est, double* J, double* wt, hipStream_t s);
diff --git a/vinsat_amd/csrc/vba_obs.hip b/vinsat_amd/csrc/vba_obs.hip
--- a/vinsat_amd/csrc/vba_obs.hip
+++ b/vinsat_amd/csrc/vba_obs.hip
@@ -1,4 +1,5 @@
 #include "vba_decide.h"
+#include <algorithm>
 #include <cstdlib>
 #include "vba_device.h"
 #include "vba_dyn_body.h"
@@ -1260,12 +1261,22 @@
     if (m >= 0) m_arr[w] = m;
 }
 
-__global__ void k_reset_calls(DevView V) {
-    const int w = blockIdx.x * 64 + threadIdx.x;
-    if (w < V.W) {
+__global__ __launch_bounds__(256) void k_reset_calls(DevView V, const double* stage, int n10, int clear0) {
+    const int t = blockIdx.x * 256 + threadIdx.x;
+    const int stride = gridDim.x * 256;
+    for (int w = t; w < V.W; w += stride) {
         V.sc[w].call_idx = 0;
         V.sc[w].pending = -1;
         V.sc[w].miss = 0;
+    }
+    if (stage) {
+        const double2* src = reinterpret_cast<const double2*>(stage);
+        double2* dst = reinterpret_cast<double2*>(V.states);
+        for (int k = t; k < n10 / 2; k += stride) dst[k] = src[k];
+        if (t == 0) V.sc[0].lam[V.par] = stage[n10];
+    }
+    if (clear0) {
+        for (int64_t k = t; k < (int64_t)V.W * kSelBins; k += stride) hist0_of(V, (int)(k / kSelBins), V.par)[k % kSelBins] = 0u;
     }
 }
 
@@ -1288,8 +1299,12 @@
     hipLaunchKernelGGL(k_set_counts, dim3(1), dim3(1), 0, s, const_cast<int*>(V.n), const_cast<int*>(V.m), w, n, m);
 }
 
-void launch_reset_calls(const DevView& V, hipStream_t s) {
-    hipLaunchKernelGGL(k_reset_calls, dim3((V.W + 63) / 64), dim3(64), 0, s, V);
+void launch_reset_calls(const DevView& V, hipStream_t s, const double* stage, int n10, int clear0) {
+    int64_t items = V.W;
+    if (stage) items = std::max<int64_t>(items, n10 / 2);
+    if (clear0) items = std::max<int64_t>(items, (int64_t)V.W * kSelBins);
+    const int nb = (int)std::min<int64_t>((items + 255) / 256, 1024);
+    hipLaunchKernelGGL(k_reset_calls, dim3(nb), dim3(256), 0, s, V, stage, n10, clear0);
 }
 
 void launch_broadcast_states(const DevView& V, int n, double lamda, hipStream_t s) {
diff --git a/vinsat_amd/csrc/vba_schedule.hip b/vinsat_amd/csrc/vba_schedule.hip
--- a/vinsat_amd/csrc/vba_schedule.hip
+++ b/vinsat_amd/csrc/vba_schedule.hip
@@ -309,7 +309,8 @@
 
 int vba_run_schedule(vba_handle h, int ncalls, const int* iters, const int* inits, int* trials_total) {
     if (!h || !iters || !inits || ncalls < 1) return fail(VBA_EINVAL, "bad argument");
-    if (int rc_settle = settle(h)) return rc_settle;
+    VBA_ESTAMP(3);
+    if (int rc_settle = settle(h, false, true)) return rc_settle;
     if (int rc = ready(h)) return rc;
     HIPCHK(hipSetDevice(h->device));
     hipStream_t s = h->stream;
@@ -330,18 +331,17 @@
         q.fold = fold;
         return q;
     };
-    {
-        DevView V0;
-        view_for_call(h, V0, spec(0, false));
-        if (h->need_hist_reset) {
-            DevView Q = V0;
-            for (int p = 0; p < 2; ++p) { Q.par = p; launch_clear_hist(Q, 1, s); }
-            h->need_hist_reset = false;
-            h->hist_dirty = false;
-        }
-        if (!carry0 && h->hist_dirty) launch_clear_hist(V0, 0, s);
-        launch_reset_calls(V0, s);
-    }
+    if (h->need_hist_reset) {
+        DevView Q;
+        view_for_call(h, Q, spec(0, false));
+        for (int p = 0; p < 2; ++p) { Q.par = p; launch_clear_hist(Q, 1, s); }
+        h->need_hist_reset = false;
+        h->hist_dirty = false;
+    }
+    const int clear0 = carry0 ? 0 : 1;
+    if (h->pend.on && h->pend.par != par0) { if (int rc = flush_states(h)) return rc; }
+    const int up_n10 = h->pend.on ? h->pend.n * 10 : 0;
+    if (h->pend.on) { h->pend.on = false; h->stage_kernel = true; }
     h->hist_dirty = emit_kind != 0;
     for (int w = 0; w < h->W; ++w) { h->h_head[w].call_idx = 0; h->h_head[w].done = 0; h->h_head[w].flags = 0; }
     long trials = 0;
@@ -361,12 +361,23 @@
         std::vector<unsigned long long> gkey;
         std::vector<unsigned char> gviews;
         if (!no_graph && h->graph_enabled && guard == 0 && !prof_pass && h->V.lat && !h->graph_broken && next == 0 && (h->fusion & 96) == 0) {
-            gkey.reserve(8 + 3 * (size_t)ncalls);
+            std::vector<unsigned long long>& ident = h->ident_now;
+            ident.clear();
+            ident.push_back(h->gen); ident.push_back((unsigned long long)ncalls); ident.push_back((unsigned long long)par0);
+            ident.push_back((unsigned long long)carry0); ident.push_back((unsigned long long)emit_kind); ident.push_back((unsigned long long)(uintptr_t)s);
+            ident.push_back((unsigned long long)clear0); ident.push_back((unsigned long long)up_n10);
+            for (int c = 0; c < ncalls; ++c) ident.push_back(((unsigned long long)(unsigned)iters[c] << 1) | (inits[c] ? 1ull : 0ull));
+            size_t hit = h->graphs.size();
+            for (size_t k = 0; k < h->graphs.size(); ++k)
+                if (h->graphs[k].ident == ident) { hit = k; break; }
+            if (hit == h->graphs.size()) {
+            gkey.reserve(9 + 3 * (size_t)ncalls);
             gviews.resize((size_t)ncalls * sizeof(DevView));
             gkey.push_back((unsigned long long)ncalls); gkey.push_back((unsigned long long)par0); gkey.push_back((unsigned long long)carry0);
             gkey.push_back((unsigned long long)emit_kind); gkey.push_back((unsigned long long)h->pivot_mode);
             gkey.push_back((unsigned long long)h->inline_select | ((unsigned long long)h->fold_enabled << 1));
             gkey.push_back((unsigned long long)(uintptr_t)s);
+            gkey.push_back((unsigned long long)clear0 | ((unsigned long long)up_n10 << 1));
             for (int c = 0; c < ncalls; ++c) {
                 const bool fold = c > 0 && emit_kind == 2 && h->fold_enabled;
                 DevView Vc;
@@ -383,12 +394,15 @@
                 }
                 gkey.push_back(hsh); gkey.push_back((unsigned long long)iters[c]); gkey.push_back((unsigned long long)inits[c]);
             }
-            size_t hit = h->graphs.size();
             for (size_t k = 0; k < h->graphs.size(); ++k)
-                if (h->graphs[k].key == gkey && h->graphs[k].views == gviews) { hit = k; break; }
+                if (h->graphs[k].key == gkey && h->graphs[k].views == gviews) { hit = k; h->graphs[k].ident = ident; break; }
+            }
             if (hit < h->graphs.size()) {
                 if (hit != 0) std::rotate(h->graphs.begin(), h->graphs.begin() + hit, h->graphs.begin() + hit + 1);
-                if (hipGraphLaunch(h->graphs[0].exec, s) == hipSuccess) { replayed = true; h->graph_replays++; }
+                VBA_ESTAMP(4);
+                const hipError_t launched = hipGraphLaunch(h->graphs[0].exec, s);
+                VBA_ESTAMP(5);
+                if (launched == hipSuccess) { replayed = true; h->graph_replays++; }
                 else { (void)hipGetLastError(); h->graph_broken = true; }
             } else {
                 if (hipStreamBeginCapture(s, hipStreamCaptureModeRelaxed) == hipSuccess) capturing = true;
@@ -407,6 +421,11 @@
             }
         } capture_guard{s, &capturing};
         auto enqueue_pass = [&]() -> int {
+        if (next == 0 && !replayed) {
+            DevView V0;
+            view_for_call(h, V0, spec(0, false));
+            launch_reset_calls(V0, s, up_n10 ? h->d_stage_map : nullptr, up_n10, clear0);
+        }
         for (int c = next; c < ncalls && !replayed; ++c) {
             const bool fold = c > next && emit_kind == 2 && h->fold_enabled;
             const CallSpec q = spec(c, fold);
@@ -452,6 +471,7 @@
             }
             vba_context::GraphEntry ge;
             ge.key = gkey;
+            ge.ident = h->ident_now;
             ge.views = std::move(gviews);
             ge.exec = exec;
             h->graphs.insert(h->graphs.begin(), std::move(ge));
@@ -460,6 +480,7 @@
         }
         HIPCHK(hipGetLastError());
         if (int rc = read_heads(h)) return rc;
+        h->stage_kernel = false;
         trials += (long)(ncalls - next);
         std::vector<int> stalled, stall_at((size_t)h->W);
         for (int w = 0; w < h->W; ++w) {
@@ -515,6 +536,7 @@
 int vba_set_schedule_graph(vba_handle h, int on) {
     if (!h) return fail(VBA_EINVAL, "null handle");
     if (int rc = settle(h)) return rc;
+    h->touch();
     h->graph_enabled = on != 0;
     return VBA_OK;
 }
@@ -529,6 +551,7 @@
 int vba_set_chain_profile(vba_handle h, int on) {
     if (!h) return fail(VBA_EINVAL, "null handle");
     if (int rc = settle(h)) return rc;
+    h->touch();
     h->cprof.on = on != 0;
     return VBA_OK;
 }
@@ -664,6 +687,7 @@
 static int iterate_pipelined(vba_handle h, int iter, int initialize, double* states_out, double* lamda_out, double* last_hessian,
                              int* n_trials, unsigned* flags) {
     if (int rc = ready(h)) return rc;
+    if (int rc = flush_states(h)) return rc;
     HIPCHK(hipSetDevice(h->device));
     hipStream_t s = h->stream;
     constexpr int emit_kind = 2;
diff --git a/vinsat_amd/csrc/vba_sharded_api.hip b/vinsat_amd/csrc/vba_sharded_api.hip
--- a/vinsat_amd/csrc/vba_sharded_api.hip
+++ b/vinsat_amd/csrc/vba_sharded_api.hip
@@ -13,6 +13,7 @@
 int vba_sh_stage1(vba_handle h, int iter, int initialize, int64_t m_total, double* d_abs_local) {
     if (!h || !d_abs_local || m_total < 1) return fail(VBA_EINVAL, "bad argument");
     if (int rc_settle = settle(h)) return rc_settle;
+    h->touch();
     if (h->W != 1) return fail(VBA_EINVAL, "sharded mode uses a single window per handle");
     if (h->reg) return fail(VBA_EINVAL, "sharded mode does not take a prior (vba_set_prior)");
     if (int rc = ready(h)) return rc;
@@ -131,6 +132,7 @@
 int vba_sh_comm_init(vba_handle h, const char* rccl_path, const void* id128, int nranks, int rank) {
     if (!h || !rccl_path || !id128 || nranks < 1 || rank < 0 || rank >= nranks) return fail(VBA_EINVAL, "bad argument");
     if (int rc_settle = settle(h)) return rc_settle;
+    h->touch();
     if (h->W != 1) return fail(VBA_EINVAL, "sharded mode uses a single window per handle");
     if (h->shc.comm) return fail(VBA_ESTATE, "the handle has a communicator already");
     h->sharded = true;
@@ -211,6 +213,7 @@
         const int shift = keys <= 300000 ? 44 : (keys <= 600000 ? 43 : 42);
         if (h->V.warm_shift != shift) {
             h->V.warm_shift = shift;
+            h->touch();
             h->carry_ok = 0;
             S.carried = false;
         }
@@ -380,6 +383,7 @@
 int vba_sh_set_protocol(vba_handle h, int carried_keys) {
     if (!h) return fail(VBA_EINVAL, "null handle");
     if (int rc = settle(h)) return rc;
+    h->touch();
     h->shc.protocol = carried_keys ? 1 : 0;
     h->shc.carried = false;
     return VBA_OK;
@@ -399,6 +403,7 @@
     auto& S = h->shc;
     if (!S.comm) return fail(VBA_ESTATE, "vba_sh_comm_init has not run");
     if (int rc_settle = settle(h)) return rc_settle;
+    h->touch();
     if (h->W != 1) return fail(VBA_EINVAL, "sharded mode uses a single window per handle");
     if (h->reg) return fail(VBA_EINVAL, "sharded mode does not take a prior (vba_set_prior)");
     if (int rc = ready(h)) return rc;
```

After: 23870 BA iterations/s, median of 6. +2.9%, better.
